# uber-research/vargp

Measured on AMD Instinct MI355X. Metric: ELBO steps/sec, higher is better.
Workload: dtype f32; 1 GPU; BASELINE config 2 (Split-MNIST t=0): S3 F10 C10 M100 D784 B512 ELBO step; S_per_gpu=3, Mt=100, S_total=3, F=10, C=10, M=100, D=784, B=512, N=12000, optimizer=yogi, parallelism=sample-parallel x1, steps_per_graph_launch=10, launch=hipGraph replay

## Files before the change

vargp_amd/csrc/elbo_t0.hip:

```cpp
#include <atomic>
#include <mutex>
#include <unordered_map>

#include "common.h"
STEP_SPAN_TABLE(t0)
#include "elbo_shared.h"
#include "t0_bwd_mid.h"
#include "t0_bwd_mid_multi.h"
#include "chol_gram.h"
#include "t0_prologue.h"
#include "t0_bwd_tail.h"

namespace vargp {

constexpr int kKuuSplit = 2;
#ifndef VARGP_KL_ROWS
#define VARGP_KL_ROWS 8
#endif
constexpr int kT0TileUnitsMax = 16384;
constexpr int kTailLdsDefault = 1;
constexpr int kKlRows = VARGP_KL_ROWS;


struct T0Ws {
  float* queue;
  float *theta, *eps_theta, *eps_f, *w, *g2, *kd, *na, *nb, *xs, *Lu, *KS, *LL, *TT, *RK, *QP, *W, *mu, *var;
  float *gmu, *gvar;
  float *r_uf, *c_uf, *gtheta;
  float *r_uu, *gW, *gkd, *gQP, *gLL, *gTT, *gRK, *gKS, *Wuu, *Puu, *Puf;
  float* kpart;
  void* chol;
  size_t chol_bytes;
  int NR, LD;
  int64_t Dp;
  size_t bytes;
};

static T0Ws carve_t0(void* ws, int S, int C, int M, int D, int B, int F) {
  T0Ws o{};
  o.NR = (int)round_up(4 + 2 * M, 4);
  o.LD = (int)round_up(o.NR + B, 4);
  o.Dp = round_up(D, 4);
  const int64_t SC = (int64_t)S * C, MM = (int64_t)M * M, D1 = D + 1;
  float* p = reinterpret_cast<float*>(ws);
  auto take = [&](int64_t n) { float* q = p; p += round_up(n, 64); return q; };
  o.theta = take(S * D1); o.eps_theta = take(S * D1); o.eps_f = take((int64_t)S * F * C * B);
  o.w = take(S * o.Dp); o.g2 = take(S); o.kd = take(SC); o.queue = take(8);
  o.na = take(SC * M); o.nb = take((int64_t)S * B);
  o.xs = take((int64_t)S * B * D);
  o.Lu = take(C * MM); o.KS = take((SC + C) * MM); o.LL = take((SC + C) * MM); o.TT = take((SC + C) * MM);
  o.RK = take(SC * M * o.LD); o.QP = take(SC * M * o.LD); o.W = take(SC * M * B);
  o.mu = take(SC * B); o.var = take(SC * B);
  o.gmu = take(SC * B); o.gvar = take(SC * B);
  o.r_uf = take(SC * M); o.c_uf = take((int64_t)S * B); o.gtheta = take(S * D1);
  o.r_uu = take(SC * M); o.gW = take(SC * M * B); o.gkd = take(SC);
  o.gQP = take(SC * M * o.LD); o.gLL = take((SC + C) * MM); o.gTT = take((SC + C) * MM);
  o.gRK = take(SC * M * o.LD); o.gKS = take((SC + C) * MM); o.Wuu = take(SC * MM);
  o.Puu = take(SC * M * D); o.Puf = take(SC * M * D);
  o.kpart = o.gRK;
  const size_t cb = vargp_chol_workspace_bytes((int)(SC + C), M, 0), cbb = vargp_chol_workspace_bytes((int)(SC + C), M, 1);
  o.chol_bytes = cb > cbb ? cb : cbb;
  o.chol = p;
  p += round_up((int64_t)(o.chol_bytes + 3) / 4, 64);
  o.bytes = (size_t)((char*)p - (char*)ws);
  return o;
}

__global__ __launch_bounds__(256) void t0_prologue_kernel(const ProArgs a) {
  __shared__ float red[4];
  t0_prologue_body(a, blockIdx.x, red);
}

__global__ __launch_bounds__(256) void t0_norm_kernel(const float* __restrict__ z, const float* __restrict__ x,
                                                      const float* __restrict__ w, float* __restrict__ na,
                                                      float* __restrict__ nb, int64_t zrows, int64_t xrows, int D,
                                                      int64_t Dp) {
  const int64_t row = (int64_t)blockIdx.x * 4 + (threadIdx.x >> 6);
  const int s = blockIdx.y, lane = threadIdx.x & 63;
  if (row >= zrows + xrows) return;
  const bool isz = row < zrows;
  const float* xr = isz ? z + row * D : x + (row - zrows) * D;
  const float* ws = w + s * Dp;
  const float acc = row_norm_wave(xr, ws, D, lane);
  if (lane == 0) {
    if (isz) na[(int64_t)s * zrows + row] = acc; else nb[(int64_t)s * xrows + (row - zrows)] = acc;
  }
}

__global__ __launch_bounds__(256) void t0_combine_norm_kernel(const float* __restrict__ part, int nsplit, int64_t sSplit,
                                                              const float* __restrict__ g2, float* __restrict__ Kuu, int C,
                                                              int M, int64_t total, int ncomb, const float* __restrict__ z,
                                                              const float* __restrict__ x, const float* __restrict__ w,
                                                              float* __restrict__ na, float* __restrict__ nb,
                                                              int64_t zrows, int64_t xrows, int D, int64_t Dp, int nrow4) {
  if ((int)blockIdx.x < ncomb) {
    const int64_t e = (int64_t)blockIdx.x * 256 + threadIdx.x;
    if (e >= total) return;
    const int j = e % M, i = (e / M) % M;
    const int64_t b = e / ((int64_t)M * M);
    const int64_t base = b * M * M;
    float gij = 0.f, gii = 0.f, gjj = 0.f;
    for (int k0 = 0; k0 < nsplit; k0 += 4) {
      float vij[4], vii[4], vjj[4];
#pragma unroll
      for (int q = 0; q < 4; ++q) {
        const float* pk = part + min(k0 + q, nsplit - 1) * sSplit + base;
        vij[q] = pk[(int64_t)i * M + j]; vii[q] = pk[(int64_t)i * M + i]; vjj[q] = pk[(int64_t)j * M + j];
      }
#pragma unroll
      for (int q = 0; q < 4; ++q) {
        if (k0 + q < nsplit) { gij += vij[q]; gii += vii[q]; gjj += vjj[q]; }
      }
    }
    const float gam = g2[b / C];
    Kuu[e] = i == j ? gam : gam * expf(-0.5f * (gii + gjj - 2.f * gij));
    return;
  }
  const int id = (int)blockIdx.x - ncomb;
  const int64_t row = (int64_t)(id % nrow4) * 4 + (threadIdx.x >> 6);
  const int s = id / nrow4, lane = threadIdx.x & 63;
  if (row >= zrows + xrows) return;
  const bool isz = row < zrows;
  const float* xr = isz ? z + row * D : x + (row - zrows) * D;
  const float* ws = w + s * Dp;
  const float acc = row_norm_wave(xr, ws, D, lane);
  if (lane == 0) {
    if (isz) na[(int64_t)s * zrows + row] = acc; else nb[(int64_t)s * xrows + (row - zrows)] = acc;
  }
}

__global__ void t0_pack_kernel(const float* __restrict__ m, const float* __restrict__ LS, const float* __restrict__ Lu,
                               float* __restrict__ RK, int C, int M, int NR, int LD, int64_t total) {
  const int64_t e = (int64_t)blockIdx.x * blockDim.x + threadIdx.x;
  if (e >= total) return;
  const int col = e % NR;
  const int64_t row = e / NR;
  const int i = row % M;
  const int64_t c = (row / M) % C;
  float v = 0.f;
  if (col == 0) v = m[c * M + i];
  else if (col >= 4 && col < 4 + M) v = LS[(c * M + i) * M + (col - 4)];
  else if (col >= 4 + M && col < 4 + 2 * M) v = Lu[(c * M + i) * M + (col - 4 - M)];
  RK[row * LD + col] = v;
}

__global__ __launch_bounds__(256) void t0_pdiag_kl_fwd_kernel(const float* __restrict__ QP, const float* __restrict__ W,
                                                              const float* __restrict__ kd, const float* __restrict__ Lz,
                                                              const float* __restrict__ Lu, float* __restrict__ mu,
                                                              float* __restrict__ var, float* __restrict__ kl_u, int S,
                                                              int C, int M, int B, int NR, int LD, int nbx, int npd,
                                                              int nkx, uint32_t* rng_counter) {
  __shared__ float red[3][4][64];
  if (rng_counter && blockIdx.x == 0 && threadIdx.x == 0) rng_counter[0] += 1u;
  if ((int)blockIdx.x < npd) {
    const int cx = threadIdx.x & 63, ry = threadIdx.x >> 6;
    const int col = ((int)blockIdx.x % nbx) * 64 + cx;
    const int64_t b = blockIdx.x / nbx;
    float m0 = 0.f, d1 = 0.f, d2 = 0.f;
    if (col < B) {
      const float* q = QP + b * M * LD;
      const float* p = q + NR + col;
      const float* w = W + b * M * B + col;
#pragma unroll 4
      for (int m = ry; m < M; m += 4) {
        const float pv = p[(int64_t)m * LD], wv = w[(int64_t)m * B];
        m0 = fmaf(pv, q[(int64_t)m * LD], m0);
        d1 = fmaf(pv, pv, d1);
        d2 = fmaf(wv, wv, d2);
      }
    }
    red[0][ry][cx] = m0; red[1][ry][cx] = d1; red[2][ry][cx] = d2;
    __syncthreads();
    if (ry == 0 && col < B) {
      m0 = red[0][0][cx] + red[0][1][cx] + red[0][2][cx] + red[0][3][cx];
      d1 = red[1][0][cx] + red[1][1][cx] + red[1][2][cx] + red[1][3][cx];
      d2 = red[2][0][cx] + red[2][1][cx] + red[2][2][cx] + red[2][3][cx];
      mu[b * B + col] = m0;
      var[b * B + col] = kd[b] - d1 + d2;
    }
    return;
  }
  const int id = (int)blockIdx.x - npd;
  const int64_t b = id / nkx;
  const int c = b % C;
  const int i0 = (id % nkx) * kKlRows, i1 = min(M, i0 + kKlRows);
  const float* q = QP + b * M * LD;
  float acc = 0.f;
  for (int e = threadIdx.x; e < (i1 - i0) * M; e += 256) {
    const int i = i0 + e / M, j = e % M;
    if (j <= i) { const float v = q[(int64_t)i * LD + 4 + M + j]; acc = fmaf(v, v, acc); }
  }
  for (int i = i0 + threadIdx.x; i < i1; i += 256) {
    const float a = q[(int64_t)i * LD];
    acc = fmaf(a, a, acc);
    acc += 2.f * (logf(Lz[(b * M + i) * M + i]) - logf(Lu[((int64_t)c * M + i) * M + i])) - 1.f;
  }
  const float t = block_sum<256>(acc, &red[0][0][0]);
  if (threadIdx.x == 0) atomicAdd(kl_u, 0.5f * t / (float)S);
}

constexpr int kFusedTS = 108;
constexpr int kFusedGS = 132;
constexpr int kFusedKS = 68;
constexpr int kFusedK = 104;
constexpr size_t kFusedLdsBytes = sizeof(float) * (128 * kFusedTS + kFusedK * kFusedGS + kFusedK * kFusedKS + 128 + 3 * 64);
typedef float f32x16_t __attribute__((ext_vector_type(16)));
#ifdef FF_STAMPS
__device__ unsigned long long g_ff_stamps[4][16];
extern "C" void vargp_debug_ff_stamps(unsigned long long* out) { (void)hipMemcpyFromSymbol(out, HIP_SYMBOL(g_ff_stamps), sizeof(g_ff_stamps)); }
#ifndef FF_STAMP_BLOCK
#define FF_STAMP_BLOCK 0u
#endif
#define FF_STAMP(i) do { if ((threadIdx.x & 63) == 0 && blockIdx.x == (FF_STAMP_BLOCK)) g_ff_stamps[threadIdx.x >> 6][i] = __builtin_amdgcn_s_memtime(); } while (0)
#else
#define FF_STAMP(i) do { } while (0)
#endif

__device__ __forceinline__ void ff_mfma4x2(f32x16_t& x, f32x16_t& y, const float4 a, const float4 c, const float4 b) {
  x = __builtin_amdgcn_mfma_f32_32x32x2f32(a.x, b.x, x, 0, 0, 0);
  y = __builtin_amdgcn_mfma_f32_32x32x2f32(c.x, b.x, y, 0, 0, 0);
  x = __builtin_amdgcn_mfma_f32_32x32x2f32(a.y, b.y, x, 0, 0, 0);
  y = __builtin_amdgcn_mfma_f32_32x32x2f32(c.y, b.y, y, 0, 0, 0);
  x = __builtin_amdgcn_mfma_f32_32x32x2f32(a.z, b.z, x, 0, 0, 0);
  y = __builtin_amdgcn_mfma_f32_32x32x2f32(c.z, b.z, y, 0, 0, 0);
  x = __builtin_amdgcn_mfma_f32_32x32x2f32(a.w, b.w, x, 0, 0, 0);
  y = __builtin_amdgcn_mfma_f32_32x32x2f32(c.w, b.w, y, 0, 0, 0);
}
__device__ __forceinline__ void ff_mfma4(f32x16_t& x, const float4 a, const float4 b) {
  x = __builtin_amdgcn_mfma_f32_32x32x2f32(a.x, b.x, x, 0, 0, 0);
  x = __builtin_amdgcn_mfma_f32_32x32x2f32(a.y, b.y, x, 0, 0, 0);
  x = __builtin_amdgcn_mfma_f32_32x32x2f32(a.z, b.z, x, 0, 0, 0);
  x = __builtin_amdgcn_mfma_f32_32x32x2f32(a.w, b.w, x, 0, 0, 0);
}
template <int R0, int R1>
__device__ __forceinline__ void ff_product_p(f32x16_t (&acc)[2], const float* __restrict__ sT, const float* __restrict__ sK, int cb,
                                             int li, int lh) {
  constexpr int GE = kFusedK / 8, G0 = bm_min(GE, 4 * R0 + 4), G1 = bm_min(GE, 4 * R1 + 4);
  const float* arow0 = sT + (32 * R0 + li) * kFusedTS + 4 * lh;
  const float* arow1 = sT + (32 * R1 + li) * kFusedTS + 4 * lh;
  const float* bcol = sK + (4 * lh) * kFusedKS + 32 * cb + li;
  float4 a0 = bm_frag_kc(arow0, 0), a1 = bm_frag_kc(arow1, 0), bb = bm_frag_km(bcol, 0, kFusedKS);
  bm_for<0, G1>([&](auto gi) {
    constexpr int g = decltype(gi)::value;
    const float4 c0 = a0, c1 = a1, cbv = bb;
    if constexpr (g + 1 < G1) {
      if constexpr (g + 1 < G0) a0 = bm_frag_kc(arow0, 8 * (g + 1));
      a1 = bm_frag_kc(arow1, 8 * (g + 1));
      bb = bm_frag_km(bcol, 8 * (g + 1), kFusedKS);
    }
    if constexpr (g < G0) ff_mfma4x2(acc[0], acc[1], c0, c1, cbv);
    else ff_mfma4(acc[1], c1, cbv);
  });
}
template <int R0, int R1>
__device__ __forceinline__ void ff_product_w(f32x16_t (&acc)[2], const float* __restrict__ sG, const float* __restrict__ sK, int cb,
                                             int li, int lh) {
  constexpr int GE = kFusedK / 8, S0 = 4 * R0, S1 = 4 * R1;
  const float* acol0 = sG + (4 * lh) * kFusedGS + 32 * R0 + li;
  const float* acol1 = sG + (4 * lh) * kFusedGS + 32 * R1 + li;
  const float* bcol = sK + (4 * lh) * kFusedKS + 32 * cb + li;
  float4 a0 = bm_frag_km(acol0, 8 * S0, kFusedGS), a1 = a0, bb = bm_frag_km(bcol, 8 * S0, kFusedKS);
  bm_for<S0, GE>([&](auto gi) {
    constexpr int g = decltype(gi)::value;
    const float4 c0 = a0, c1 = a1, cbv = bb;
    if constexpr (g + 1 < GE) {
      a0 = bm_frag_km(acol0, 8 * (g + 1), kFusedGS);
      if constexpr (g + 1 >= S1) a1 = bm_frag_km(acol1, 8 * (g + 1), kFusedGS);
      bb = bm_frag_km(bcol, 8 * (g + 1), kFusedKS);
    }
    if constexpr (g >= S1) ff_mfma4x2(acc[0], acc[1], c0, c1, cbv);
    else ff_mfma4(acc[0], c0, cbv);
  });
}

template <bool MULTI>
__device__ __forceinline__ void ff_barrier() {
  if constexpr (MULTI) bmm_lds_barrier(); else __syncthreads();
}
template <bool VEC4, bool MULTI = false>
__global__ __launch_bounds__(256) void t0_fwd_fused_kernel(const float* __restrict__ TT, float* __restrict__ QP,
                                                           const float* __restrict__ RK, float* __restrict__ W,
                                                           const float* __restrict__ kd, const float* __restrict__ Lz,
                                                           const float* __restrict__ Lu, float* __restrict__ mu,
                                                           float* __restrict__ var, float* __restrict__ kl_u, int S, int C,
                                                           int M, int B, int NR, int LD, int ntile, uint32_t* rng_counter,
                                                           int nparts) {
  extern __shared__ __attribute__((aligned(16))) float lds_f[];
  STEP_SPAN(t0, 3);
  float* sT = lds_f;
  float* sG = sT + 128 * kFusedTS;
  float* sK = sG + kFusedK * kFusedGS;
  float* sa = sK + kFusedK * kFusedKS;
  float* red = sa + 128;
  const int tid = threadIdx.x, lane = tid & 63, wave = tid >> 6, li = lane & 31, lh = lane >> 5;
  const int xcd = (int)blockIdx.x & 7, idx = (int)blockIdx.x >> 3;
  const int64_t b = (int64_t)(idx / nparts) * 8 + xcd;
  const int64_t MM = (int64_t)M * M, MLD = (int64_t)M * LD;
  if (rng_counter && blockIdx.x == 0 && tid == 0) rng_counter[0] += 1u;
  if (b >= (int64_t)S * C) return;
  const int part = idx % nparts;
  int tile_x = MULTI ? (part * ntile) / nparts : part;
  const int tile_end = MULTI ? ((part + 1) * ntile) / nparts : part + 1;
  int n0 = tile_x * 64;
  const float* Tb = TT + b * MM;
  const float* Qb = QP + b * MLD;
  const float* Kb = RK + b * MLD + NR;
  FF_STAMP(0);
  FF_STAMP(1);
  constexpr int NT_ = 128 * (kFusedK / 4) / 256;
  constexpr int NG_ = kFusedK * 32 / 256;
  constexpr int NK_ = (kFusedK * 16 + 255) / 256;
  float4 rt[NT_], rg[NG_], rk[NK_];
  const char* Tbb = reinterpret_cast<const char*>(Tb);
  const char* Qbb = reinterpret_cast<const char*>(Qb);
  const char* Kbb = reinterpret_cast<const char*>(Kb);
#pragma unroll
  for (int u = 0; u < NT_; ++u) {
    const int e = tid + 256 * u;
    const int i = e / (kFusedK / 4), k = (e - i * (kFusedK / 4)) * 4;
    const int ic = min(i, M - 1);
    rt[u] = *reinterpret_cast<const float4*>(Tbb + 4u * (__umul24((unsigned)ic, (unsigned)M) + (unsigned)min(k, min(M - 4, ic & ~3))));
  }
#pragma unroll
  for (int u = 0; u < NG_; ++u) {
    const int e = tid + 256 * u;
    const int k = e >> 5, i = (e & 31) * 4;
    const int kc = min(k, M - 1);
    rg[u] = *reinterpret_cast<const float4*>(Qbb + 4u * (__umul24((unsigned)kc, (unsigned)LD) + 4u + (unsigned)min(i, min(M - 4, kc & ~3))));
  }
  auto load_ktile = [&](const int n0_) {
    const char* Kt = Kbb + 4 * n0_;
#pragma unroll
    for (int u = 0; u < NK_; ++u) {
      const int e = min(tid + 256 * u, kFusedK * 16 - 1);
      const int k = e >> 4, n = (e & 15) * 4;
      const unsigned ro = 4u * __umul24((unsigned)min(k, M - 1), (unsigned)LD);
      if constexpr (VEC4) {
        rk[u] = *reinterpret_cast<const float4*>(Kt + ro + 4u * (unsigned)min(n, B - 4 - n0_));
      } else {
        const float* src = reinterpret_cast<const float*>(Kt + ro);
        rk[u].x = n0_ + n < B ? src[n] : 0.f;         rk[u].y = n0_ + n + 1 < B ? src[n + 1] : 0.f;
        rk[u].z = n0_ + n + 2 < B ? src[n + 2] : 0.f; rk[u].w = n0_ + n + 3 < B ? src[n + 3] : 0.f;
      }
    }
  };
  load_ktile(n0);
  const float av = tid < 128 ? *reinterpret_cast<const float*>(Qbb + 4u * __umul24((unsigned)min(tid, M - 1), (unsigned)LD)) : 0.f;
  const int c_kl = b % C;
  const int per = (M + nparts - 1) / nparts, i0 = part * per, i1 = min(M, i0 + per);
  const int nkl = max((i1 - i0) * M, 0);
  const unsigned mdiv = ((1u << 20) + (unsigned)M - 1u) / (unsigned)M;
  float kv[8];
#pragma unroll
  for (int u = 0; u < 8; ++u) {
    const int e = min(tid + 256 * u, max(nkl - 1, 0));
    const int ei = (int)(((unsigned)e * mdiv) >> 20);
    kv[u] = *reinterpret_cast<const float*>(Qbb + 4u * (__umul24((unsigned)min(i0 + ei, M - 1), (unsigned)LD) + 4u + (unsigned)M + (unsigned)(e - ei * M)));
  }
  const int idg = min(i0 + tid, M - 1);
  const float dga = *reinterpret_cast<const float*>(Qbb + 4u * __umul24((unsigned)idg, (unsigned)LD));
  const float dlz = Lz[(b * M + idg) * M + idg], dlu = Lu[((int64_t)c_kl * M + idg) * M + idg];
  FF_STAMP(10);
#pragma unroll
  for (int u = 0; u < NT_; ++u) {
    const int e = tid + 256 * u;
    const int i = e / (kFusedK / 4), k = (e - i * (kFusedK / 4)) * 4;
    const bool ok = i < M && k < M && k <= i;
    *reinterpret_cast<float4*>(&sT[i * kFusedTS + k]) = ok ? rt[u] : make_float4(0.f, 0.f, 0.f, 0.f);
  }
  FF_STAMP(11);
#pragma unroll
  for (int u = 0; u < NG_; ++u) {
    const int e = tid + 256 * u;
    const int k = e >> 5, i = (e & 31) * 4;
    *reinterpret_cast<float4*>(&sG[k * kFusedGS + i]) = (k < M && i < M && i <= k) ? rg[u] : make_float4(0.f, 0.f, 0.f, 0.f);
  }
  if (tid < 128) sa[tid] = tid < M ? av : 0.f;
  if (tid < 192) red[tid] = 0.f;
  float kl_acc = 0.f;
#pragma unroll
  for (int u = 0; u < 8; ++u) {
    const int e = tid + 256 * u;
    const int ei = (int)(((unsigned)e * mdiv) >> 20);
    const int i = i0 + ei, j = e - ei * M;
    kl_acc = fmaf((e < nkl && j <= i) ? kv[u] : 0.f, kv[u], kl_acc);
  }
  for (int e0 = 8 * 256; e0 < nkl; e0 += 8 * 256) {
#pragma unroll
    for (int u = 0; u < 8; ++u) {
      const int e = min(e0 + tid + 256 * u, nkl - 1);
      kv[u] = Qb[(int64_t)(i0 + e / M) * LD + 4 + M + e % M];
    }
#pragma unroll
    for (int u = 0; u < 8; ++u) {
      const int e = e0 + tid + 256 * u;
      const int i = i0 + e / M, j = e % M;
      kl_acc = fmaf((e < nkl && j <= i) ? kv[u] : 0.f, kv[u], kl_acc);
    }
  }
  {
    const bool dok = i0 + tid < i1;
    float t = fmaf(dga, dga, 2.f * (logf(dlz) - logf(dlu)) - 1.f);
    kl_acc += dok ? t : 0.f;
    for (int i = i0 + tid + 256; i < i1; i += 256) {
      const float a = Qb[(int64_t)i * LD];
      kl_acc = fmaf(a, a, kl_acc);
      kl_acc += 2.f * (logf(Lz[(b * M + i) * M + i]) - logf(Lu[((int64_t)c_kl * M + i) * M + i])) - 1.f;
    }
  }
  do {
#pragma unroll
  for (int u = 0; u < NK_; ++u) {
    const int e = tid + 256 * u;
    if (e < kFusedK * 16) {
      const int k = e >> 4, n = (e & 15) * 4;
      *reinterpret_cast<float4*>(&sK[k * kFusedKS + n]) = (k < M && (!VEC4 || n0 + n < B)) ? rk[u] : make_float4(0.f, 0.f, 0.f, 0.f);
    }
  }
  FF_STAMP(12);
  if constexpr (MULTI) { if (tile_x + 1 < tile_end) load_ktile(n0 + 64); }
  FF_STAMP(13);
  ff_barrier<MULTI>();
  FF_STAMP(2);
  if constexpr (MULTI) {
    const int l16 = lane & 15, q = lane >> 4, n = 16 * wave + l16, col = n0 + n;
    bm_f32x4 accP[kB16NB];
#pragma unroll
    for (int i = 0; i < kB16NB; ++i)
#pragma unroll
      for (int r = 0; r < 4; ++r) accP[i][r] = 0.f;
    b16_prod<true, kFusedTS>(sT, sK, wave, l16, q, accP);
    ff_barrier<true>();
    float s_mu = 0.f, s_p2 = 0.f, s_w2 = 0.f;
    char* Pout_b = reinterpret_cast<char*>(QP + b * MLD + NR);
#pragma unroll
    for (int i = 0; i < kB16NB; ++i) {
      float sav[4];
#pragma unroll
      for (int r = 0; r < 4; ++r) sav[r] = sa[16 * i + 4 * q + r];
#pragma unroll
      for (int r = 0; r < 4; ++r) {
        const int m = 16 * i + 4 * q + r;
        const float v = m < M ? accP[i][r] : 0.f;
        if (m < kFusedK) sK[m * kFusedKS + n] = v;
        if (m < M && col < B) *reinterpret_cast<float*>(Pout_b + 4u * (__umul24((unsigned)m, (unsigned)LD) + (unsigned)col)) = v;
        s_mu = fmaf(v, sav[r], s_mu);
        s_p2 = fmaf(v, v, s_p2);
      }
    }
    ff_barrier<true>();
    char* Wb_b = reinterpret_cast<char*>(W + b * (int64_t)M * B);
    bm_f32x4 accW[kB16NB];
#pragma unroll
    for (int i = 0; i < kB16NB; ++i)
#pragma unroll
      for (int r = 0; r < 4; ++r) accW[i][r] = 0.f;
    b16_prod<false, kFusedGS>(sG, sK, wave, l16, q, accW);
#pragma unroll
    for (int i = 0; i < kB16NB; ++i)
#pragma unroll
      for (int r = 0; r < 4; ++r) {
        const int m = 16 * i + 4 * q + r;
        if (m < M) {
          const float v = accW[i][r];
          if (col < B) *reinterpret_cast<float*>(Wb_b + 4u * (__umul24((unsigned)m, (unsigned)B) + (unsigned)col)) = v;
          s_w2 = fmaf(v, v, s_w2);
        }
      }
    s_mu += __shfl_xor(s_mu, 16, 64); s_p2 += __shfl_xor(s_p2, 16, 64); s_w2 += __shfl_xor(s_w2, 16, 64);
    s_mu += __shfl_xor(s_mu, 32, 64); s_p2 += __shfl_xor(s_p2, 32, 64); s_w2 += __shfl_xor(s_w2, 32, 64);
    if (q == 0) { red[n] = s_mu; red[64 + n] = s_p2; red[128 + n] = s_w2; }
    ff_barrier<true>();
    if (tid < 64 && n0 + tid < B) {
      mu[b * B + n0 + tid] = red[tid];
      var[b * B + n0 + tid] = kd[b] - red[64 + tid] + red[128 + tid];
    }
    tile_x += 1; n0 += 64;
  } else {
  const int cb = wave & 1;
  const int rbs[2] = {(wave >> 1) ? 1 : 0, (wave >> 1) ? 2 : 3};
  f32x16_t accP[2];
#pragma unroll
  for (int u = 0; u < 2; ++u)
#pragma unroll
    for (int r = 0; r < 16; ++r) accP[u][r] = 0.f;
  if ((wave >> 1) == 0) ff_product_p<0, 3>(accP, sT, sK, cb, li, lh);
  else ff_product_p<1, 2>(accP, sT, sK, cb, li, lh);
  FF_STAMP(3);
  ff_barrier<MULTI>();
  FF_STAMP(4);
  const int col = n0 + 32 * cb + li;
  float s_mu = 0.f, s_p2 = 0.f, s_w2 = 0.f;
  char* Pout_b = reinterpret_cast<char*>(QP + b * MLD + NR);
#pragma unroll
  for (int u = 0; u < 2; ++u) {
    float sav[16];
#pragma unroll
    for (int r = 0; r < 16; ++r) sav[r] = sa[32 * rbs[u] + (r & 3) + 8 * (r >> 2) + 4 * lh];
#pragma unroll
    for (int r = 0; r < 16; ++r) {
      const int m = 32 * rbs[u] + (r & 3) + 8 * (r >> 2) + 4 * lh;
      const float v = accP[u][r];
      if (m < kFusedK) sK[m * kFusedKS + 32 * cb + li] = v;
      if (m < M && col < B) *reinterpret_cast<float*>(Pout_b + 4u * (__umul24((unsigned)m, (unsigned)LD) + (unsigned)col)) = v;
      s_mu = fmaf(v, sav[r], s_mu);
      s_p2 = fmaf(v, v, s_p2);
    }
  }
  ff_barrier<MULTI>();
  FF_STAMP(5);
  char* Wb_b = reinterpret_cast<char*>(W + b * (int64_t)M * B);
  {
    const int rlo = min(rbs[0], rbs[1]), rhi = max(rbs[0], rbs[1]);
    f32x16_t accW[2];
#pragma unroll
    for (int u = 0; u < 2; ++u)
#pragma unroll
      for (int r = 0; r < 16; ++r) accW[u][r] = 0.f;
    if ((wave >> 1) == 0) ff_product_w<0, 3>(accW, sG, sK, cb, li, lh);
    else ff_product_w<1, 2>(accW, sG, sK, cb, li, lh);
    FF_STAMP(6);
#pragma unroll
    for (int u = 0; u < 2; ++u) {
      const int rb = u ? rhi : rlo;
#pragma unroll
      for (int r = 0; r < 16; ++r) {
        const int m = 32 * rb + (r & 3) + 8 * (r >> 2) + 4 * lh;
        if (m < M) {
          const float v = accW[u][r];
          if (col < B) *reinterpret_cast<float*>(Wb_b + 4u * (__umul24((unsigned)m, (unsigned)B) + (unsigned)col)) = v;
          s_w2 = fmaf(v, v, s_w2);
        }
      }
    }
  }
  FF_STAMP(7);
  s_mu += __shfl_xor(s_mu, 32, 64); s_p2 += __shfl_xor(s_p2, 32, 64); s_w2 += __shfl_xor(s_w2, 32, 64);
  if (lh == 0) {
    atomicAdd(&red[32 * cb + li], s_mu); atomicAdd(&red[64 + 32 * cb + li], s_p2); atomicAdd(&red[128 + 32 * cb + li], s_w2);
  }
  ff_barrier<MULTI>();
  if (tid < 64) {
    if (n0 + tid < B) {
      mu[b * B + n0 + tid] = red[tid];
      var[b * B + n0 + tid] = kd[b] - red[64 + tid] + red[128 + tid];
    }
  }
  FF_STAMP(8);
  }
  } while (MULTI && tile_x < tile_end);
  __syncthreads();
  const float tkl = block_sum<256>(kl_acc, red);
  if (tid == 0) atomicAdd(kl_u, 0.5f * tkl / (float)S);
  FF_STAMP(9);
}

__global__ __launch_bounds__(256) void t0_bwd_head_kernel(const float* __restrict__ QP, const float* __restrict__ W,
                                                          const float* __restrict__ gmu, const float* __restrict__ gvar,
                                                          const float* __restrict__ gscale, const float* __restrict__ Lz,
                                                          const float* __restrict__ seeds, float* __restrict__ gQP,
                                                          float* __restrict__ gW, float* __restrict__ gkd,
                                                          float* __restrict__ gLz, float* __restrict__ gThead,
                                                          float* __restrict__ gTtail, float* __restrict__ zero_begin, int64_t zero_count, int S, int C,
                                                          int M, int B, int NR, int LD, int npd, int nkx, int nkl, int fused,
                                                          float* __restrict__ g_u_mean, float* __restrict__ gLu_acc) {
  __shared__ float red[4];
  const float g = seeds[1] / (float)S;
  if ((int)blockIdx.x < npd) {
    const int m = (int)blockIdx.x % M;
    const int64_t b = blockIdx.x / M;
    const int64_t offp = (b * M + m) * LD + NR, offw = (b * M + m) * B;
    const float am = QP[(b * M + m) * LD];
    const float gs = gscale ? gscale[0] : 1.f;
    float acc = 0.f, accv = 0.f;
    for (int c0 = 0; c0 < B; c0 += 1024) {
      float gm[4], gv[4], pv[4], wv[4];
#pragma unroll
      for (int q = 0; q < 4; ++q) {
        const int col = min(c0 + 256 * q + (int)threadIdx.x, B - 1);
        gm[q] = gmu[b * B + col]; gv[q] = gvar[b * B + col];
        pv[q] = QP[offp + col]; wv[q] = W[offw + col];
      }
#pragma unroll
      for (int q = 0; q < 4; ++q) {
        const int col = c0 + 256 * q + (int)threadIdx.x;
        if (col < B) {
          const float m_ = gs * gm[q], v_ = gs * gv[q];
          gQP[offp + col] = am * m_ - 2.f * pv[q] * v_;
          gW[offw + col] = 2.f * wv[q] * v_;
          acc = fmaf(pv[q], m_, acc);
          accv += v_;
        }
      }
    }
    const float t = block_sum<256>(acc, red);
    if (threadIdx.x == 0) gQP[(b * M + m) * LD] = t + g * am;
    if (m == 0) {
      const float tv = block_sum<256>(accv, red);
      if (threadIdx.x == 0) gkd[b] = tv;
    }
    return;
  }
  const int id = (int)blockIdx.x - npd;
  if (id >= nkl) {
    const int nz = gridDim.x - npd - nkl;
    for (int64_t i = (int64_t)(id - nkl) * 256 + threadIdx.x; i < zero_count; i += (int64_t)nz * 256) zero_begin[i] = 0.f;
    return;
  }
  const int64_t b = id / nkx;
  const int s = b / C, c = b % C;
  const int i0 = (id % nkx) * kKlRows, i1 = min(M, i0 + kKlRows);
  const float* q = QP + b * M * LD;
  float* gq = gQP + b * M * LD;
  const int nel = (i1 - i0) * M;
  for (int e00 = 0; e00 < nel; e00 += 1024) {
    float qv[4], lv[4];
#pragma unroll
    for (int u = 0; u < 4; ++u) {
      const int e0 = min(e00 + 256 * u + (int)threadIdx.x, nel - 1);
      const int i = i0 + e0 / M, j = e0 % M;
      qv[u] = q[(int64_t)i * LD + 4 + M + j];
      lv[u] = Lz[b * M * M + i * M + j];
    }
#pragma unroll
    for (int u = 0; u < 4; ++u) {
      const int e0 = e00 + 256 * u + (int)threadIdx.x;
      if (e0 < nel) {
        const int i = i0 + e0 / M, j = e0 % M;
        const int e = i * M + j;
        gq[(int64_t)i * LD + 4 + M + j] = (j <= i) ? g * qv[u] : 0.f;
        gq[(int64_t)i * LD + 4 + j] = 0.f;
        gThead[b * M * M + e] = 0.f;
        gLz[b * M * M + e] = (i == j) ? g / lv[u] : 0.f;
        if (s == 0) {
          gTtail[(int64_t)c * M * M + e] = 0.f;
          if (gLu_acc) gLu_acc[(int64_t)c * M * M + e] = 0.f;
        }
      }
    }
  }
  for (int i = i0 + threadIdx.x; i < i1; i += 256) {
    if (fused) gq[(int64_t)i * LD] = g * q[(int64_t)i * LD];
    if (g_u_mean && s == 0) g_u_mean[(int64_t)c * M + i] = 0.f;
    gq[(int64_t)i * LD + 1] = 0.f; gq[(int64_t)i * LD + 2] = 0.f; gq[(int64_t)i * LD + 3] = 0.f;
    for (int col = 4 + 2 * M; col < NR; ++col) gq[(int64_t)i * LD + col] = 0.f;
  }
  if (fused && i0 == 0 && threadIdx.x == 0) gkd[b] = 0.f;
}

__global__ void t0_unpack_kernel(const float* __restrict__ gRK, float* __restrict__ g_u_mean, float* __restrict__ gLS,
                                 int S, int C, int M, int LD, int64_t total) {
  const int64_t e = (int64_t)blockIdx.x * blockDim.x + threadIdx.x;
  if (e >= total) return;
  const int jj = e % (M + 1);
  const int64_t ci = e / (M + 1);
  const int col = jj == 0 ? 0 : 3 + jj;
  float acc = 0.f;
  for (int s0 = 0; s0 < S; s0 += 8) {
    float t[8];
#pragma unroll
    for (int u = 0; u < 8; ++u) t[u] = gRK[((int64_t)min(s0 + u, S - 1) * C * M + ci) * LD + col];
#pragma unroll
    for (int u = 0; u < 8; ++u) acc += (s0 + u < S) ? t[u] : 0.f;
  }
  if (jj == 0) g_u_mean[ci] = acc; else gLS[ci * M + (jj - 1)] = acc;
}

static int ensure_dynamic_lds(const void* fn, size_t bytes, std::atomic<unsigned> (&mask)[2], const char* who) {
  int dev = 0;
  VARGP_REQUIRE(hipGetDevice(&dev) == hipSuccess && dev >= 0 && dev < 64, "%s: hipGetDevice failed", who);
  if (!((mask[dev >> 5].load(std::memory_order_acquire) >> (dev & 31)) & 1u)) {
    VARGP_REQUIRE(hipFuncSetAttribute(fn, hipFuncAttributeMaxDynamicSharedMemorySize, (int)bytes) == hipSuccess,
                  "%s: cannot reserve %zu bytes of LDS", who, bytes);
    mask[dev >> 5].fetch_or(1u << (dev & 31), std::memory_order_release);
  }
  return VARGP_OK;
}

static bool t0_native(const vargp_elbo_t0_desc* d) { return d->eps_f == nullptr && !d->ext_lik; }
static int check_desc(const vargp_elbo_t0_desc* d, const char* who) {
  VARGP_REQUIRE(d, "%s: null descriptor", who);
  VARGP_REQUIRE(d->S > 0 && d->C > 0 && d->M > 0 && d->D > 0 && d->B > 0 && d->F > 0, "%s: bad dims", who);
  VARGP_REQUIRE(d->log_mean && d->z && d->u_mean && d->u_tril_vec && d->x && (d->y || d->ext_lik) && d->scalars && d->info && d->ws,
                "%s: null pointer", who);
  const bool native = t0_native(d);
  VARGP_REQUIRE(!native || (d->rng_counter && d->eps_theta == nullptr && d->rng_sample_offset >= 0),
                "%s: native noise needs rng_counter, eps_theta == eps_f == NULL and a sample offset >= 0", who);
  VARGP_REQUIRE(d->map_est ? d->S == 1
                           : (d->log_logvar && d->prior_log_mean && d->prior_log_logvar && (native || d->eps_theta)),
                "%s: hyper-parameter arguments inconsistent with map_est", who);
  VARGP_REQUIRE(d->ws_bytes >= vargp_elbo_t0_workspace_bytes(d->S, d->C, d->M, d->D, d->B, d->F),
                "%s: workspace too small", who);
  return VARGP_OK;
}

struct T0Tune {
  static long long env(const char* name, long long dflt) { const char* e = getenv(name); return e ? atoll(e) : dflt; }
  int64_t units = env("VARGP_T0_UNITS", kT0TileUnitsMax);
  int unmerge = env("VARGP_T0_UNMERGE", -1), side = env("VARGP_T0_SIDE", 1);
  int multi = env("VARGP_T0_MULTI", 0), parts = env("VARGP_T0_PARTS", 0);
  int fused = env("VARGP_T0_FUSED", 1), fused_bwd = env("VARGP_T0_FUSED_BWD", 1), mat_bwd = env("VARGP_T0_MAT_BWD", 1);
  int front = env("VARGP_T0_FRONT", 1), gram_in_chain = env("VARGP_T0_GRAM_IN_CHAIN", -1), su = env("VARGP_T0_SU", 1);
  int tail = env("VARGP_T0_TAIL", 1), tail_lds = env("VARGP_T0_TAIL_LDS", kTailLdsDefault);
  int kuf_tile = env("VARGP_T0_KUF_TILE", 0), puf_tile = env("VARGP_T0_PUF_TILE", 0), puu_tile = env("VARGP_T0_PUU_TILE", 0);
  int kuu_split = env("VARGP_KUU_SPLIT", kKuuSplit), chol_f32 = env("VARGP_CHOL_F32", kCholF32Default);
};
static const T0Tune& t0_tune() { static const T0Tune tune; return tune; }

constexpr float kFwdMidSetup = 0.5f;
constexpr float kBwdMidSetup = 0.35f;
static int t0_tile_parts(int64_t SC, int ntile, int cus, float setup, int forced) {
  if (forced > 0) return forced < ntile ? forced : ntile;
  if (SC * ntile <= cus) return ntile;
  int best = ntile;
  float best_t = 1e30f;
  for (int np = 1; np <= ntile; ++np) {
    const float t = (float)cdiv(SC * np, (int64_t)cus) * (setup + (float)cdiv(ntile, np));
    if (t < best_t - 1e-6f) { best_t = t; best = np; }
  }
  return best;
}

struct T0Plan {
  bool native, generic_lik, unscaled_lik_grad, defer_softmax, fwd_softmax16;
  bool direct_gram, merge_chol, split_kuu, front, gram_in_chain, su_in_chain, fused_mid, fwd_multi, w_vec4;
  bool unmerge, side;
  bool fused_bwd, mat_bwd, bwd_multi, fused_tail, tail_lds;
  int kuf_tile, puf_tile, puu_tile;
  int ksp, ntile, fwd_parts, bwd_parts;
};
static T0Plan t0_plan(const vargp_elbo_t0_desc* d, const T0Ws& o, int cus) {
  const T0Tune& tune = t0_tune();
  const int S = d->S, C = d->C, M = d->M, D = d->D, B = d->B, F = d->F, LD = o.LD;
  const int64_t SC = (int64_t)S * C;
  const bool zx_aligned = ((reinterpret_cast<uintptr_t>(d->z) | reinterpret_cast<uintptr_t>(d->x)) & 15) == 0;
  T0Plan p{};
  p.native = t0_native(d);
  p.unscaled_lik_grad = C <= 16 && !d->ext_lik;
  p.generic_lik = C > 16 && !d->ext_lik;
  p.ntile = cdiv(B, 64);
  p.kuf_tile = tune.kuf_tile; p.puf_tile = tune.puf_tile; p.puu_tile = tune.puu_tile;

  p.direct_gram = D <= kRbfDirectD;
  p.merge_chol = D > kRbfDirectD && M > 50 && M <= 100 && (D % 4) == 0 && (LD % 4) == 0 && zx_aligned;
  p.ksp = tune.kuu_split;
  p.split_kuu = p.merge_chol && D >= 256 && (int64_t)p.ksp * M <= LD && p.ksp > 1;
  p.front = p.split_kuu && tune.front && p.ksp <= kCholPartMax && D <= kProKuuMaxD;

  p.unmerge = SC + C >= (tune.unmerge >= 0 ? tune.unmerge : cus / 3 + 1);
  p.side = p.unmerge && tune.side != 0;

  p.gram_in_chain = p.front && (tune.gram_in_chain >= 0 ? S >= tune.gram_in_chain : p.unmerge) && M > 64 && (M % 4) == 0 &&
                    D <= kCgMaxD && D >= 32;
  p.su_in_chain = VARGP_CHOL_BLK16 && tune.su && tune.chol_f32 && p.merge_chol && M > 64 && (M % 4) == 0 && M <= 100;

  const bool units_ok = SC * p.ntile <= tune.units;
  p.fused_mid = tune.fused && M <= kFusedK && (M % 4) == 0 && (LD % 4) == 0 && units_ok;
  p.fwd_parts = t0_tile_parts(SC, p.ntile, cus, kFwdMidSetup, tune.parts);
  p.fwd_multi = p.fwd_parts < p.ntile || tune.multi == 1;
  p.w_vec4 = B % 4 == 0;
  p.fused_bwd = tune.fused_bwd && M <= kBmKP && M >= 4 && (M % 4) == 0 && (LD % 4) == 0 && (B % 4) == 0 && units_ok;
  p.mat_bwd = p.fused_bwd && tune.mat_bwd && (D % 4) == 0 && S <= kTailSMax && zx_aligned;
  p.bwd_parts = t0_tile_parts(SC, p.ntile, cus, kBwdMidSetup, tune.parts);
  p.bwd_multi = p.fused_bwd && (p.bwd_parts < p.ntile || tune.multi == 1);
  p.defer_softmax = d->defer_softmax && p.unscaled_lik_grad && p.fused_bwd && !p.bwd_multi && F <= 4 * kBmSmF && C <= kBmSmC &&
                    reinterpret_cast<uintptr_t>(p.native ? o.eps_f : d->eps_f) % 16 == 0;
  p.fwd_softmax16 = p.unscaled_lik_grad && !p.defer_softmax;
  p.fused_tail = p.mat_bwd && tune.tail && S <= kTailSMax;
  p.tail_lds = p.fused_tail && ((S > 4 && tune.tail_lds) || tune.tail_lds == 2);
  return p;
}

enum { kT0NoClear = 0, kT0Cleared = 1, kT0Consumed = 2, kT0SoftmaxDeferred = 16  };
static std::mutex g_t0_state_mu;
static std::unordered_map<const void*, int> g_t0_state;
static void t0_state_set(const void* ws, int v) {
  std::lock_guard<std::mutex> lock(g_t0_state_mu);
  if (g_t0_state.size() > 4096) {
    for (auto it = g_t0_state.begin(); it != g_t0_state.end();)
      it = ((it->second & 15) == kT0Cleared && it->first != ws) ? std::next(it) : g_t0_state.erase(it);
  }
  g_t0_state[ws] = v;
}
static int t0_state_get(const void* ws) {
  std::lock_guard<std::mutex> lock(g_t0_state_mu);
  auto it = g_t0_state.find(ws);
  return it == g_t0_state.end() ? -1 : it->second;
}

struct T0 {
  const vargp_elbo_t0_desc* d;
  T0Ws o;
  T0Plan plan;
  vargp_stream_t stream;
  hipStream_t st;
  int S, C, M, D, B, F, SC, NR, LD;
  int64_t MM, MLD, zrows;
  const float *eps_f, *eps_theta;

  T0(const vargp_elbo_t0_desc* d_, vargp_stream_t stream_)
      : d(d_), o(carve_t0(d_->ws, d_->S, d_->C, d_->M, d_->D, d_->B, d_->F)), plan(t0_plan(d_, o, vargp_cu_count())),
        stream(stream_), st(as_stream(stream_)), S(d_->S), C(d_->C), M(d_->M), D(d_->D), B(d_->B), F(d_->F), SC(d_->S * d_->C),
        NR(o.NR), LD(o.LD), MM((int64_t)d_->M * d_->M), MLD((int64_t)d_->M * o.LD), zrows((int64_t)d_->C * d_->M),
        eps_f(plan.native ? o.eps_f : d_->eps_f), eps_theta(plan.native ? o.eps_theta : d_->eps_theta) {}

  GemmParams kuu_gemm() const {
    GemmParams p = flat_gemm(d->z, D, 0, d->z, D, 0, o.KS, M, C * MM, M, M, D);
    p.nb1 = C; p.sA[1] = (int64_t)M * D; p.sB[1] = (int64_t)M * D; p.sC[1] = MM;
    p.kscale = o.w; p.ks_ld = o.Dp; p.g2 = o.g2;
    p.na = o.na; p.sNa[0] = zrows; p.sNa[1] = M;
    p.nbv = o.na; p.sNb[0] = zrows; p.sNb[1] = M;
    p.same_xy = 1;
    return p;
  }
  GemmParams kuf_gemm(bool prescaled) const {
    GemmParams p = flat_gemm(d->z, D, 0, d->x, D, 0, o.RK + NR, LD, (int64_t)C * MLD, C * M, B, D);
    p.kscale = o.w; p.ks_ld = o.Dp; p.g2 = o.g2;
    p.na = o.na; p.sNa[0] = zrows;
    p.nbv = o.nb; p.sNb[0] = B;
    if (prescaled) { p.B = o.xs; p.sB[0] = (int64_t)B * D; p.kscale = nullptr; }
    return p;
  }
  ElboGemm qp_gemm(int ncols) const {
    ElboGemm g{flat_gemm(o.TT, M, MM, o.RK, LD, MLD, o.QP, LD, MLD, M, ncols, M), 0, 0, SC, ncols == NR ? "t0_qps_gemm" : "t0_qp_gemm"};
    g.p.triA = 1;
    return g;
  }
  ElboGemm gt_gemm(bool small) const {
    ElboGemm g{flat_gemm(o.gQP, LD, MLD, o.RK, LD, MLD, o.gTT, M, MM, M, M, small ? NR : NR + B), 0, 1, SC, "t0_gt_gemm"};
    g.p.triC = 1;
    if (small) return g.onto_c();
    g.p.splitk = ksplit(NR + B);
    return g;
  }
  ElboGemm grk_gemm(int ncols) const {
    ElboGemm g{flat_gemm(o.TT, M, MM, o.gQP, LD, MLD, o.gRK, LD, MLD, M, ncols, M), 1, 0, SC, "t0_grk_gemm"};
    g.p.triA = 2;
    return g;
  }
  GemmParams puu_gemm() const {
    GemmParams p = flat_gemm(o.Wuu, M, C * MM, d->z, D, 0, o.Puu, D, zrows * D, M, D, M);
    p.nb1 = C; p.sA[1] = MM; p.sB[1] = (int64_t)M * D; p.sC[1] = (int64_t)M * D;
    return p;
  }
  GemmParams puf_gemm() const { return flat_gemm(o.gRK + NR, LD, C * MLD, d->x, D, 0, o.Puf, D, zrows * D, C * M, D, B); }
  int fwd() const;
  int bwd(const float* seeds, float* g_log_mean, float* g_log_logvar, float* g_z, float* g_u_mean, float* g_u_tril_vec) const;
};

int T0::fwd() const {
  int rc;
  t0_state_set(d->ws, (plan.mat_bwd ? kT0Cleared : kT0NoClear) | (plan.defer_softmax ? kT0SoftmaxDeferred : 0));
  ZeroJobs bwd_zero{};
  if (plan.mat_bwd) {
    bwd_zero.j[0] = ZeroJob{o.gQP, (int64_t)SC * M, 4 + M, LD};
    bwd_zero.j[1] = ZeroJob{o.gTT, 1, (SC + C) * MM, 0};
    bwd_zero.j[2] = ZeroJob{o.queue, 1, 8, 0};
    bwd_zero.j[3] = ZeroJob{o.gkd, 1, SC, 0};
    bwd_zero.j[4] = ZeroJob{o.r_uf, 1, o.r_uu - o.r_uf, 0};
    if (plan.unmerge)
      bwd_zero.j[5] = ZeroJob{o.gLL + SC * MM, 1, C * MM, 0};
  }
  ProArgs a{};
  if (plan.merge_chol) { a.RK = o.RK; a.u_mean = d->u_mean; a.NR = NR; a.LD = LD; }
  a.mean = d->log_mean; a.logvar = d->log_logvar; a.pmean = d->prior_log_mean; a.plogvar = d->prior_log_logvar;
  a.eps_theta = d->eps_theta; a.vec = d->u_tril_vec;
  a.theta = o.theta; a.w = o.w; a.g2 = o.g2; a.kd = o.kd; a.Lu = o.Lu; a.Su = o.KS + SC * MM; a.scalars = d->scalars;
  a.bump = d->bump;
  a.su_in_chain = plan.su_in_chain ? 1 : 0;
  a.zero_begin = o.gmu; a.zero_count = o.r_uf - o.gmu; a.info = d->info; a.Dp = o.Dp;
  a.S = S; a.C = C; a.M = M; a.D = D; a.ninfo = SC + C; a.map_est = d->map_est;
  a.nzero_blocks = (int)std::min<int64_t>(64, cdiv(a.zero_count, 1024));
  if (plan.native) {
    const int64_t per_sample_f = (int64_t)F * C * B;
    a.native = 1; a.seed = d->rng_seed; a.rng_counter = d->rng_counter;
    a.g0_theta = (int64_t)d->rng_sample_offset * (D + 1); a.g0_f = (int64_t)d->rng_sample_offset * per_sample_f;
    a.n_f = S * per_sample_f;
    a.eps_theta_out = o.eps_theta; a.eps_f_out = o.eps_f;
    a.nrng_blocks = (int)std::min<int64_t>(512, cdiv(a.n_f + 7, 1024));
  }
  if (plan.mat_bwd && !plan.merge_chol) {
    a.zero = bwd_zero;
    const int64_t zt = (int64_t)SC * M * (4 + M) + (SC + 2 * C) * MM + (o.r_uu - o.r_uf);
    a.nzero_blocks = (int)std::min<int64_t>(128, cdiv(a.zero_count + zt, 2048));
  }
  const int npro = 1 + S + a.nzero_blocks + a.nrng_blocks + cdiv((int64_t)C * MM, 256);
  if (!plan.front) {
    ProfScope prof("t0_prologue", st);
    hipLaunchKernelGGL(t0_prologue_kernel, dim3(npro), dim3(256), 0, st, a);
  }
  if (plan.direct_gram) {
    rc = rbf_direct_launch(d->z, nullptr, o.w, o.g2, o.KS, M, S, C, M, M, D, o.Dp, 0, st);
    if (rc) return rc;
    rc = rbf_direct_launch(d->z, d->x, o.w, o.g2, o.RK + NR, LD, S, C, M, B, D, o.Dp, 1, st);
    if (rc) return rc;
  } else {
    if (!plan.split_kuu)
      hipLaunchKernelGGL(t0_norm_kernel, dim3(cdiv(zrows + B, 4), S), dim3(256), 0, st, d->z, d->x, o.w, o.na, o.nb, zrows,
                         (int64_t)B, D, o.Dp);
    if (plan.merge_chol) {
      VARGP_REQUIRE(chol_rbf_gemm_applicable(M, kuf_gemm(false)), "elbo_t0_fwd: merged launch expected but not applicable");
      if (plan.split_kuu) {
        GemmParams ps = kuu_gemm();
        ps.splitk = plan.ksp; ps.sSplit = SC * MM; ps.C = o.kpart;
        if (plan.front) {
          NormArgs nr{d->z, d->x, o.na, o.nb, zrows, (int64_t)B, 16, (int)cdiv(zrows + B, 16), o.xs};
          rc = launch_pro_kuu(a, npro, nr, ps, plan.gram_in_chain ? 0 : SC, st);
          if (rc) return rc;
        } else {
          rc = launch_gemm(ps, 0, 1, SC, true, st, "rbf_kuu_gemm");
          if (rc) return rc;
          const int64_t total = SC * MM;
          const int ncomb = cdiv(total, 256), nrow4 = cdiv(zrows + B, 4);
          hipLaunchKernelGGL(t0_combine_norm_kernel, dim3(ncomb + nrow4 * S), dim3(256), 0, st, o.kpart, plan.ksp, SC * MM, o.g2,
                             o.KS, C, M, total, ncomb, d->z, d->x, o.w, o.na, o.nb, zrows, (int64_t)B, D, o.Dp, nrow4);
        }
      } else {
        rc = launch_gemm(kuu_gemm(), 0, 1, SC, true, st, "rbf_kuu_gemm");
        if (rc) return rc;
      }
      CholExtra lx{o.RK + 4, SC, LD, MLD, (int64_t)C * MLD, S, 1, 1};
      if (plan.front) {
        lx.part = o.kpart; lx.nsplit = plan.ksp; lx.sSplit = SC * MM; lx.g2 = o.g2; lx.part_C = C; lx.Kout = o.KS;
        if (plan.gram_in_chain) { lx.part = nullptr; lx.gram_z = d->z; lx.gram_w = o.w; lx.gram_D = D; lx.gram_Dp = o.Dp; }
      }
      if (plan.su_in_chain) lx.su_Lu = o.Lu;
      GemmParams kuf = kuf_gemm(plan.front);
      SideFork fork(st, plan.side);
      rc = launch_chol_rbf_gemm(o.KS, d->jitter, o.LL, o.TT, d->info, SC + C, M, kuf, plan.unmerge ? 0 : S, fork.side(), &lx,
                                plan.mat_bwd ? &bwd_zero : nullptr);
      if (rc) return rc;
      if (plan.unmerge) {
        kuf.tile = plan.kuf_tile;
        rc = launch_gemm(kuf, 0, 1, S, true, st, "rbf_kuf_gemm");
        if (rc) return rc;
      }
      rc = fork.join();
      if (rc) return rc;
    } else {
      rc = launch_gemm_pair(kuu_gemm(), SC, kuf_gemm(false), S, 0, 1, true, st, "rbf_kuu_gemm", "rbf_kuf_gemm");
      if (rc) return rc;
    }
  }
  if (!plan.merge_chol) {
    rc = chol_inv_fwd_impl(o.KS, d->jitter, o.LL, o.TT, nullptr, d->info, SC + C, M, o.chol, o.chol_bytes, false, st);
    if (rc) return rc;
    const int64_t total = (int64_t)SC * M * NR;
    hipLaunchKernelGGL(t0_pack_kernel, dim3(cdiv(total, 256)), dim3(256), 0, st, d->u_mean, o.LL + SC * MM, o.Lu, o.RK, C,
                       M, NR, LD, total);
  }
  if (d->info_host && d->info_event) {
    VARGP_REQUIRE(hipMemcpyAsync(d->info_host, d->info, sizeof(int32_t) * (size_t)(SC + C), hipMemcpyDeviceToHost, st) == hipSuccess &&
                      hipEventRecord(reinterpret_cast<hipEvent_t>(d->info_event), st) == hipSuccess,
                  "elbo_t0_fwd: copy / event record of the early Cholesky status failed");
  }
  uint32_t* rngc = plan.native ? d->rng_counter : nullptr;
  if (plan.fused_mid) {
    rc = qp_gemm(NR).run(st);
    if (rc) return rc;
    static std::atomic<unsigned> attr_set_mask[4][2] = {};
    const dim3 grid(8 * cdiv(SC, 8) * plan.fwd_parts);
#define VARGP_FF(V4, MT, SLOT)                                                                                                  \
  do {                                                                                                                          \
    rc = ensure_dynamic_lds(reinterpret_cast<const void*>(t0_fwd_fused_kernel<V4, MT>), kFusedLdsBytes, attr_set_mask[SLOT],    \
                            "elbo_t0_fwd");                                                                                     \
    if (rc) return rc;                                                                                                          \
    hipLaunchKernelGGL((t0_fwd_fused_kernel<V4, MT>), grid, dim3(256), kFusedLdsBytes, st, o.TT, o.QP, o.RK, o.W, o.kd, o.LL,   \
                       o.Lu, o.mu, o.var, d->scalars + 1, S, C, M, B, NR, LD, plan.ntile, rngc, plan.fwd_parts);                  \
  } while (0)
    if (plan.w_vec4) { if (plan.fwd_multi) VARGP_FF(true, true, 0); else VARGP_FF(true, false, 1); }
    else { if (plan.fwd_multi) VARGP_FF(false, true, 2); else VARGP_FF(false, false, 3); }
#undef VARGP_FF
  } else {
    rc = qp_gemm(NR + B).run(st);
    if (rc) return rc;
    ElboGemm w{flat_gemm(o.QP + 4, LD, MLD, o.QP + NR, LD, MLD, o.W, B, (int64_t)M * B, M, B, M), 1, 0, SC, "t0_w_gemm"};
    w.p.triA = 2;
    rc = w.run(st);
    if (rc) return rc;
    const int ntile = plan.ntile, npd = ntile * SC, nkx = cdiv(M, kKlRows);
    hipLaunchKernelGGL(t0_pdiag_kl_fwd_kernel, dim3(npd + nkx * SC), dim3(256), 0, st, o.QP, o.W, o.kd, o.LL, o.Lu, o.mu,
                       o.var, d->scalars + 1, S, C, M, B, NR, LD, ntile, npd, nkx, rngc);
  }
  if (plan.fwd_softmax16) {
    const int64_t total = (int64_t)S * F * B;
    hipLaunchKernelGGL(t0_softmax_kernel<16>, dim3(cdiv(total, 256)), dim3(256), 0, st, o.mu, o.var, eps_f, d->y,
                       d->scalars + 2, o.gmu, o.gvar, S, F, C, B);
  } else if (plan.generic_lik) {
    rc = vargp_softmax_nll_fwd(o.mu, o.var, eps_f, d->y, d->scalars + 2, S, F, C, B, stream);
    if (rc) return rc;
  }
  return check_launch("elbo_t0_fwd");
}

int T0::bwd(const float* seeds, float* g_log_mean, float* g_log_logvar, float* g_z, float* g_u_mean, float* g_u_tril_vec) const {
  int rc;
  const int64_t MB = (int64_t)M * B;
  const float* lik_seed = plan.unscaled_lik_grad ? seeds + 2 : nullptr;
  if (plan.generic_lik) {
    rc = vargp_softmax_nll_bwd(o.mu, o.var, eps_f, d->y, seeds + 2, o.gmu, o.gvar, S, F, C, B, stream);
    if (rc) return rc;
  }
  const int state_all = t0_state_get(d->ws);
  const bool softmax_deferred = state_all >= 0 && (state_all & kT0SoftmaxDeferred) != 0;
  VARGP_REQUIRE(!softmax_deferred || plan.fused_bwd, "elbo_t0_bwd: the forward deferred the likelihood to a backward path this call does not take");
  if (plan.mat_bwd) {
    const int state = state_all < 0 ? state_all : (state_all & ~kT0SoftmaxDeferred);
    VARGP_REQUIRE(state == kT0Cleared,
                  "elbo_t0_bwd: %s -- this path allows ONE vargp_elbo_t0_bwd per vargp_elbo_t0_fwd (the forward clears the "
                  "accumulators the backward adds into); run the forward again",
                  state == kT0Consumed ? "second backward on one forward"
                                       : "no forward on this workspace with the same z / x alignment");
    t0_state_set(d->ws, kT0Consumed);
  } else if (softmax_deferred) {
    t0_state_set(d->ws, kT0NoClear);
  }
  if (!plan.mat_bwd) {
    const int npd = plan.fused_bwd ? 0 : M * SC, nkx = cdiv(M, kKlRows), nkl = nkx * SC;
    const int64_t zc = o.r_uu - o.r_uf;
    const int nz = (int)std::min<int64_t>(64, cdiv(zc, 1024));
    hipLaunchKernelGGL(t0_bwd_head_kernel, dim3(npd + nkl + nz), dim3(256), 0, st, o.QP, o.W, o.gmu, o.gvar, lik_seed, o.LL,
                       seeds, o.gQP, o.gW, o.gkd, o.gLL, o.gTT, o.gTT + SC * MM, o.r_uf, zc, S, C, M, B, NR, LD, npd, nkx, nkl,
                       plan.fused_bwd ? 1 : 0, (float*)nullptr, (float*)nullptr);
  }
  if (plan.fused_bwd) {
    static std::atomic<unsigned> attr_set_mask[2] = {}, attr_set_mask_m[2] = {};
    float* gum = plan.mat_bwd ? g_u_mean : nullptr;
    if (plan.bwd_multi) {
      VARGP_REQUIRE(!softmax_deferred, "elbo_t0_bwd: the multi-tile backward does not evaluate a deferred likelihood");
      rc = ensure_dynamic_lds(reinterpret_cast<const void*>(t0_bwd_mid_multi_kernel), kBwdMidMultiLdsBytes, attr_set_mask_m, "elbo_t0_bwd");
      if (rc) return rc;
      ProfScope prof("t0_bwd_mid", st);
      hipLaunchKernelGGL(t0_bwd_mid_multi_kernel, dim3(8 * cdiv(SC, 8) * plan.bwd_parts), dim3(256), kBwdMidMultiLdsBytes, st, o.TT, o.QP,
                         o.W, o.RK, o.gmu, o.gvar, lik_seed, o.gQP, o.gTT, o.gRK, o.gkd, o.r_uf, o.c_uf, o.gtheta, S, C, M,
                         B, D, NR, LD, plan.ntile, plan.bwd_parts, gum, C * M);
    } else {
      const BmSoftmax smx = softmax_deferred ? BmSoftmax{o.mu, o.var, eps_f, d->y, d->scalars + 2, F} : BmSoftmax{};
      rc = ensure_dynamic_lds(reinterpret_cast<const void*>(t0_bwd_mid_kernel), kBwdMidLdsBytes, attr_set_mask, "elbo_t0_bwd");
      if (rc) return rc;
      ProfScope prof("t0_bwd_mid", st);
      hipLaunchKernelGGL(t0_bwd_mid_kernel, dim3(8 * cdiv(SC, 8) * plan.ntile), dim3(256), kBwdMidLdsBytes, st, o.TT, o.QP, o.W, o.RK, o.gmu, o.gvar,
                         lik_seed, o.gQP, o.gTT, o.gRK, o.gkd, o.r_uf, o.c_uf, o.gtheta, S, C, M, B, D,
                         NR, LD, plan.ntile, gum, C * M, smx);
    }
    if (!plan.mat_bwd) {
      rc = run_gemm_pair(gt_gemm(true), grk_gemm(NR), "t0_gt_grk_small", st);
      if (rc) return rc;
      rc = chol_inv_bwd_first(o.TT, o.gTT, SC + C, M, o.chol, o.chol_bytes, nullptr, 0, 0, 0, st);
      if (rc) return rc;
    }
  } else {
    ElboGemm gg{flat_gemm(o.QP + NR, LD, MLD, o.gW, B, MB, o.gQP + 4, LD, MLD, M, M, B), 0, 1, SC, "t0_gg_gemm"};
    gg.p.splitk = ksplit(B);
    ElboGemm gp{flat_gemm(o.QP + 4, LD, MLD, o.gW, B, MB, o.gQP + NR, LD, MLD, M, B, M), 0, 0, SC, "t0_gp_gemm"};
    gp.p.triA = 1;
    rc = run_gemm_pair(gg, gp.onto_c(), "t0_gg_gp_gemm", st);
    if (rc) return rc;
    rc = gt_gemm(false).run(st);
    if (rc) return rc;
    const ElboGemm grk = grk_gemm(NR + B);
    rc = chol_inv_bwd_first(o.TT, o.gTT, SC + C, M, o.chol, o.chol_bytes, &grk.p, grk.tA, grk.tB, grk.nbatch, st);
    if (rc) return rc;
  }
  if (plan.mat_bwd) {
    BwdMatArgs ma{};
    ma.QP = o.QP; ma.TT = o.TT; ma.LL = o.LL; ma.gQP = o.gQP; ma.RK = o.RK; ma.KS = o.KS; ma.seeds = seeds; ma.gTT = o.gTT;
    ma.gKS = o.gKS; ma.Wuu = o.Wuu; ma.r_uu = o.r_uu; ma.gtheta = o.gtheta;
    ma.g_u_mean = g_u_mean; ma.gLu_part = o.gLL;
    ma.S = S; ma.C = C; ma.M = M; ma.D = D; ma.NR = NR; ma.LD = LD;
    GemmParams puf = puf_gemm();
    if (plan.unmerge) {
      SideFork fork(st, plan.side);
      ma.gL_acc = o.gLL + SC * MM;
      rc = launch_bwdmat_gemm(ma, 0, SC, puf, 0, fork.side(), "t0_bwdmat_kuu", nullptr);
      if (rc) return rc;
      rc = launch_bwdmat_gemm(ma, SC, C, puf, 0, fork.side(), "t0_bwdmat_su", nullptr);
      if (rc) return rc;
      puf.tile = plan.puf_tile;
      rc = launch_gemm(puf, 0, 0, S, false, st, "rbf_kuf_bwd_product");
      if (rc) return rc;
      rc = fork.join();
    } else {
      rc = launch_bwdmat_gemm(ma, 0, SC + C, puf, S, st, "rbf_kuf_bwd_gemm", reinterpret_cast<int*>(o.queue));
    }
    if (rc) return rc;
    if (!plan.fused_tail) {
      GemmParams puu = puu_gemm();
      puu.tile = plan.puu_tile;
      rc = launch_gemm(puu, 0, 0, SC, false, st, "rbf_kuu_bwd_gemm");
      if (rc) return rc;
    }
  } else {
    const int64_t total = (int64_t)C * M * (M + 1);
    hipLaunchKernelGGL(t0_unpack_kernel, dim3(cdiv(total, 256)), dim3(256), 0, st, o.gRK, g_u_mean, o.gLL + SC * MM, S, C,
                       M, LD, total);
    rc = chol_inv_bwd_impl(o.LL, o.TT, o.gLL, o.gTT, o.gKS, SC + C, M, o.chol, o.chol_bytes, true, st, true);
    if (rc) return rc;
    const int gx = cdiv(B, 256), gy = cdiv(zrows, kWRows), nuf = plan.fused_bwd ? 0 : gx * gy * S;
    const int nuu = SC * cdiv(M, kUuRows);
    const int ngv = cdiv((int64_t)C * MM, 256);
    hipLaunchKernelGGL(t0_w_kernel, dim3(nuf + nuu + ngv), dim3(256), 0, st, o.RK, o.gRK, o.KS, o.gKS, o.Wuu, o.r_uu, o.r_uf,
                       o.c_uf, o.gtheta, S, C, M, B, D, NR, LD, gx, gy, nuf, nuu, d->u_tril_vec, o.Lu, seeds, g_u_tril_vec, 1);
    rc = launch_gemm_pair(puu_gemm(), SC, puf_gemm(), S, 0, 0, false, st, "rbf_kuu_bwd_gemm", "rbf_kuf_bwd_gemm");
    if (rc) return rc;
  }
  const int nzy = cdiv(zrows, kFinRows), nxy = cdiv(B, kFinRows), gx = cdiv(D, 64);
  GvecArgs gv{};
  int ngy = 0;
  if (plan.mat_bwd) {
    gv.vec = d->u_tril_vec; gv.Lu = o.Lu; gv.gSu = o.gKS + SC * MM; gv.gLu_part = o.gLL; gv.seeds = seeds;
    gv.gvec = g_u_tril_vec; gv.S = S; gv.C = C; gv.M = M; gv.y0 = nzy + nxy;
    ngy = cdiv(cdiv((int64_t)C * MM, 256), gx);
  }
  if (plan.fused_tail) {
    ProfScope prof("t0_puu_final", st);
    TailArgs ta{};
    ta.z = d->z; ta.x = d->x; ta.Wuu = o.Wuu; ta.Puf = o.Puf; ta.r_uu = o.r_uu; ta.r_uf = o.r_uf; ta.c_uf = o.c_uf; ta.w = o.w;
    ta.gz = g_z; ta.gtheta = o.gtheta; ta.S = S; ta.C = C; ta.M = M; ta.D = D; ta.B = B; ta.Dp = o.Dp;
    const int rem = M % 32;
    ta.nrb = (rem > 0 && rem <= 8) ? M / 32 : cdiv(M, 32);
    const int ngr = cdiv(M, 32);
    ta.ncb = cdiv(D, 32); ta.nz = cdiv(C * ta.nrb * ta.ncb + C * (ngr * (ngr + 1) / 2), 4);
    ta.nx = gx * cdiv(B, kTailXRows); ta.gx = gx;
    ta.nrem = (rem > 0 && rem <= 8) ? C * gx * cdiv(rem, 4) : 0;
    const dim3 grid(ta.nz + ta.nrem + ta.nx);
    if (plan.tail_lds) {
      static std::atomic<unsigned> attr_set_mask_t[2] = {};
      rc = ensure_dynamic_lds(reinterpret_cast<const void*>(t0_puu_final_lds_kernel), kTailLdsBytes, attr_set_mask_t, "elbo_t0_bwd");
      if (rc) return rc;
      const int nzg = C * ta.nrb * cdiv(ta.ncb, 4), ngvw = cdiv(C * (ngr * (ngr + 1) / 2), 4);
      hipLaunchKernelGGL(t0_puu_final_lds_kernel, dim3(nzg + ngvw + ta.nrem + ta.nx), dim3(512), kTailLdsBytes, st, ta, gv, nzg, ngvw);
    } else
    switch (S) {
      case 1: hipLaunchKernelGGL(t0_puu_final_kernel<1>, grid, dim3(256), 0, st, ta, gv); break;
      case 2: hipLaunchKernelGGL(t0_puu_final_kernel<2>, grid, dim3(256), 0, st, ta, gv); break;
      case 3: hipLaunchKernelGGL(t0_puu_final_kernel<3>, grid, dim3(256), 0, st, ta, gv); break;
      case 4: hipLaunchKernelGGL(t0_puu_final_kernel<4>, grid, dim3(256), 0, st, ta, gv); break;
      default: hipLaunchKernelGGL(t0_puu_final_kernel<0>, grid, dim3(256), 0, st, ta, gv); break;
    }
  } else {
    hipLaunchKernelGGL(t0_final_kernel, dim3(gx, nzy + nxy + ngy), dim3(256), 0, st, d->z, d->x, o.r_uu, o.r_uf, o.c_uf,
                       o.Puu, o.Puf, o.w, g_z, o.gtheta, zrows, (int64_t)B, D, o.Dp, S, nzy, gv);
  }
  if (!d->defer_hyper) {
    vargp_hyper_grad_desc h;
    hyper_grad_desc_fill(d, o, eps_theta, seeds, &h);
    hyper_bwd_launch(h, g_log_mean, g_log_logvar, st);
  }
  return check_launch("elbo_t0_bwd");
}

}

using namespace vargp;

extern "C" size_t vargp_elbo_t0_workspace_bytes(int S, int C, int M, int D, int B, int F) {
  return carve_t0(nullptr, S, C, M, D, B, F).bytes + 256;
}

extern "C" int vargp_elbo_t0_lik_buffers(const vargp_elbo_t0_desc* d, float** mu, float** var, float** gmu, float** gvar) {
  VARGP_REQUIRE(d && d->ws, "elbo_t0_lik_buffers: null pointer");
  const T0Ws o = carve_t0(d->ws, d->S, d->C, d->M, d->D, d->B, d->F);
  if (mu) *mu = o.mu;
  if (var) *var = o.var;
  if (gmu) *gmu = o.gmu;
  if (gvar) *gvar = o.gvar;
  return VARGP_OK;
}

extern "C" int vargp_elbo_t0_fwd(const vargp_elbo_t0_desc* d, vargp_stream_t stream) {
  const int rc = check_desc(d, "elbo_t0_fwd");
  return rc ? rc : T0(d, stream).fwd();
}

extern "C" int vargp_elbo_t0_bwd(const vargp_elbo_t0_desc* d, const float* seeds, float* g_log_mean, float* g_log_logvar,
                                 float* g_z, float* g_u_mean, float* g_u_tril_vec, vargp_stream_t stream) {
  const int rc = check_desc(d, "elbo_t0_bwd");
  if (rc) return rc;
  VARGP_REQUIRE(seeds && g_z && g_u_mean && g_u_tril_vec && (d->defer_hyper || (g_log_mean && g_log_logvar)),
                "elbo_t0_bwd: null pointer");
  return T0(d, stream).bwd(seeds, g_log_mean, g_log_logvar, g_z, g_u_mean, g_u_tril_vec);
}

extern "C" int vargp_elbo_t0_hyper_desc(const vargp_elbo_t0_desc* d, const float* seeds, vargp_hyper_grad_desc* out) {
  int rc = check_desc(d, "elbo_t0_hyper_desc");
  if (rc) return rc;
  VARGP_REQUIRE(seeds && out, "elbo_t0_hyper_desc: null pointer");
  const T0Ws o = carve_t0(d->ws, d->S, d->C, d->M, d->D, d->B, d->F);
  hyper_grad_desc_fill(d, o, t0_native(d) ? o.eps_theta : d->eps_theta, seeds, out);
  return VARGP_OK;
}
```

vargp_amd/csrc/t0_bwd_common.h:

```cpp
#pragma once
#include "common.h"
#include <type_traits>

namespace vargp {


constexpr int kBmKP = 104;
constexpr int kBmSA = 108;
constexpr int kBmST = 68;
constexpr size_t kBwdMidLdsBytes =
    sizeof(float) * (kBmKP * kBmSA + 2 * kBmKP * kBmST + 128  + 64 + 64  + 64  + 8 +
                     3 * 4 * 64 );
constexpr int kBmSmC = 16, kBmSmF = 4;
struct BmSoftmax {
  const float *mu, *var, *eps;
  const int64_t* y;
  float* nll;
  int F;
};
typedef float bm_f32x16 __attribute__((ext_vector_type(16)));

__device__ __forceinline__ float4 bm_frag_kc(const float* __restrict__ rowp, int k) {
  return *reinterpret_cast<const float4*>(rowp + k);
}
__device__ __forceinline__ float4 bm_frag_km(const float* __restrict__ colp, int k, int stride) {
  const float* p = colp + k * stride;
  return make_float4(p[0], p[stride], p[2 * stride], p[3 * stride]);
}
__device__ __forceinline__ void bm_mfma4(bm_f32x16& acc, const float4 a, const float4 b) {
  acc = __builtin_amdgcn_mfma_f32_32x32x2f32(a.x, b.x, acc, 0, 0, 0);
  acc = __builtin_amdgcn_mfma_f32_32x32x2f32(a.y, b.y, acc, 0, 0, 0);
  acc = __builtin_amdgcn_mfma_f32_32x32x2f32(a.z, b.z, acc, 0, 0, 0);
  acc = __builtin_amdgcn_mfma_f32_32x32x2f32(a.w, b.w, acc, 0, 0, 0);
}

__device__ __forceinline__ void bmm_lds_barrier() { asm volatile("s_waitcnt lgkmcnt(0)\n\ts_barrier" ::: "memory"); }

template <int I0, int I1, class F>
__device__ __forceinline__ void bm_for(F&& f) {
  if constexpr (I0 < I1) {
    f(std::integral_constant<int, I0>{});
    bm_for<I0 + 1, I1>(f);
  }
}
__host__ __device__ constexpr int bm_min(int a, int b) { return a < b ? a : b; }

constexpr int kBmNQ = kBmKP / 4;
constexpr int kBmNA = (kBmKP * kBmNQ + 255) / 256;

template <bool TRI = false>
__device__ __forceinline__ void bm_load_mat(const float* __restrict__ base, int ld, int M, int tid, float4 (&dst)[kBmNA]) {
  const char* bp = reinterpret_cast<const char*>(base);
#pragma unroll
  for (int u = 0; u < kBmNA; ++u) {
    const int e = min(tid + 256 * u, kBmKP * kBmNQ - 1);
    const int i = e / kBmNQ, j = (e - i * kBmNQ) * 4;
    const int ic = min(i, M - 1);
    const int jc = TRI ? min(j, min(M - 4, ic & ~3)) : min(j, M - 4);
    const unsigned off = 4u * (__umul24((unsigned)ic, (unsigned)ld) + (unsigned)jc);
    dst[u] = *reinterpret_cast<const float4*>(bp + off);
  }
}

}
```

vargp_amd/csrc/t0_bwd_mid.h:

```cpp
#pragma once
#include "t0_bwd_common.h"

namespace vargp {

template <int WV> struct BmWave {
  static constexpr int NB = WV < 2 ? 3 : 2;
  static constexpr int R0 = WV < 2 ? 0 : 1, R1 = WV < 2 ? 3 : 2, CBH = WV & 1;
  __host__ __device__ static constexpr int rb(int u) { return WV == 0 ? (u == 0 ? 0 : 1) : (WV == 1 ? 2 : 3); }
  __host__ __device__ static constexpr int cb(int u) { return WV == 0 ? (u == 2 ? 1 : 0) : (WV == 1 ? u : (WV == 2 ? u : 2 + u)); }
};

__host__ __device__ constexpr int kBmAtomSplit(int nb) { return 8 * nb; }

template <int WV>
__device__ __forceinline__ void bm_tri_mfma(const float* __restrict__ sX, const float* __restrict__ sY, int li, int lh,
                                            bm_f32x16 (&acc)[3]) {
  using W = BmWave<WV>;
  const float* xr[3];
  const float* yr[3];
#pragma unroll
  for (int u = 0; u < 3; ++u) {
#pragma unroll
    for (int r = 0; r < 16; ++r) acc[u][r] = 0.f;
    xr[u] = sX + min(32 * W::rb(u < W::NB ? u : 0) + li, kBmKP - 1) * kBmST + 4 * lh;
    yr[u] = sY + min(32 * W::cb(u < W::NB ? u : 0) + li, kBmKP - 1) * kBmST + 4 * lh;
  }
#pragma unroll
  for (int k = 0; k < 64; k += 8) {
#pragma unroll
    for (int u = 0; u < W::NB; ++u) bm_mfma4(acc[u], bm_frag_kc(xr[u], k), bm_frag_kc(yr[u], k));
  }
}
template <int WV, int A>
__device__ __forceinline__ void bm_tri_atomic(const bm_f32x16 (&acc)[3], float* __restrict__ dst, int ldd, int M, int li, int lh) {
  using W = BmWave<WV>;
  constexpr int u = A / 16, r = A % 16, rb = W::rb(u), cb = W::cb(u);
  constexpr int rl = (r & 3) + 8 * (r >> 2);
  if (32 * rb + rl < M) {
    const int row = 32 * rb + rl + 4 * lh, col = 32 * cb + li;
    const bool ok = row < M && (rb != cb || col <= row);
#ifndef BM_EXP_NOATOM
#ifdef BM_EXP_PLAIN_STORES
    if (ok) dst[(int64_t)row * ldd + col] = acc[u][r];
#else
    if (ok) atomicAdd(&dst[(int64_t)row * ldd + col], acc[u][r]);
#endif
#else
    if (ok && acc[u][r] == 12345.f) dst[(int64_t)row * ldd + col] = 0.f;
#endif
  }
}

template <int WV>
__device__ __forceinline__ void bm_phase2(const float* __restrict__ sA, const float* __restrict__ sP, const float* __restrict__ sW,
                                          const float* __restrict__ sa, const float* __restrict__ sgm,
                                          const float* __restrict__ sgv, float* __restrict__ dst, int ldd, int M, int li, int lh,
                                          bm_f32x16 (&accP)[2], bm_f32x16 (&acc)[3]) {
  using W = BmWave<WV>;
  bm_tri_mfma<WV>(sP, sW, li, lh, acc);
  constexpr int R[2] = {W::R0, W::R1};
  const int n = 32 * W::CBH + li;
  {
    const float gmn = sgm[n], gvn = sgv[n];
#pragma unroll
    for (int u = 0; u < 2; ++u)
#pragma unroll
      for (int r = 0; r < 16; ++r) {
        const int m = 32 * R[u] + (r & 3) + 8 * (r >> 2) + 4 * lh;
        const int mc = min(m, kBmKP - 1);
        accP[u][r] = m < kBmKP ? fmaf(sa[mc], gmn, -2.f * sP[mc * kBmST + n] * gvn) : 0.f;
      }
  }
  constexpr int G0 = bm_min(kBmKP, 32 * W::R0 + 32) / 8, G1 = bm_min(kBmKP, 32 * W::R1 + 32) / 8;
  constexpr int NAT = kBmAtomSplit(W::NB), PER = (NAT + G1 - 1) / G1;
  const float* arow0 = sA + min(32 * W::R0 + li, kBmKP - 1) * kBmSA + 4 * lh;
  const float* arow1 = sA + min(32 * W::R1 + li, kBmKP - 1) * kBmSA + 4 * lh;
  const float* bcol = sW + (4 * lh) * kBmST + n;
  float4 nb = bm_frag_km(bcol, 0, kBmST), na0 = bm_frag_kc(arow0, 0), na1 = bm_frag_kc(arow1, 0);
  bm_for<0, G1>([&](auto gi) {
    constexpr int g = decltype(gi)::value;
    const float4 bb = nb, a0 = na0, a1 = na1;
    if constexpr (g + 1 < G1) {
      nb = bm_frag_km(bcol, 8 * (g + 1), kBmST);
      na1 = bm_frag_kc(arow1, 8 * (g + 1));
      if constexpr (g + 1 < G0) na0 = bm_frag_kc(arow0, 8 * (g + 1));
    }
    bm_mfma4(accP[1], a1, bb);
    if constexpr (g < G0) bm_mfma4(accP[0], a0, bb);
    bm_for<g * PER, bm_min((g + 1) * PER, NAT)>([&](auto ai) { bm_tri_atomic<WV, decltype(ai)::value>(acc, dst, ldd, M, li, lh); });
    __builtin_amdgcn_sched_barrier(0);
  });
}

template <int WV>
__device__ __forceinline__ void bm_phase4(const float* __restrict__ sA, const float* __restrict__ sP, const float* __restrict__ sW,
                                          float* __restrict__ dst, int ldd, int M, int li, int lh, bm_f32x16 (&accK)[2],
                                          const bm_f32x16 (&prev)[3], float* __restrict__ dprev, int ldprev, bm_f32x16 (&acc)[3]) {
  using W = BmWave<WV>;
  {
    const float* xr[3];
    const float* yr[3];
#pragma unroll
    for (int u = 0; u < 3; ++u) {
#pragma unroll
      for (int r = 0; r < 16; ++r) acc[u][r] = 0.f;
      xr[u] = sP + min(32 * W::rb(u < W::NB ? u : 0) + li, kBmKP - 1) * kBmST + 4 * lh;
      yr[u] = sW + min(32 * W::cb(u < W::NB ? u : 0) + li, kBmKP - 1) * kBmST + 4 * lh;
    }
    constexpr int A0 = kBmAtomSplit(W::NB), A1 = 16 * W::NB, PERP = (A1 - A0 + 7) / 8;
    bm_for<0, 8>([&](auto gi) {
      constexpr int g = decltype(gi)::value;
#pragma unroll
      for (int u = 0; u < W::NB; ++u) bm_mfma4(acc[u], bm_frag_kc(xr[u], 8 * g), bm_frag_kc(yr[u], 8 * g));
      bm_for<A0 + g * PERP, bm_min(A0 + (g + 1) * PERP, A1)>(
          [&](auto ai) { bm_tri_atomic<WV, decltype(ai)::value>(prev, dprev, ldprev, M, li, lh); });
    });
  }
#pragma unroll
  for (int u = 0; u < 2; ++u)
#pragma unroll
    for (int r = 0; r < 16; ++r) accK[u][r] = 0.f;
  constexpr int GS0 = 4 * W::R0, GS1 = 4 * W::R1, GE = kBmKP / 8;
  constexpr int NIT = GE - GS0, NAT = kBmAtomSplit(W::NB), PER = (NAT + NIT - 1) / NIT;
  const int n = 32 * W::CBH + li;
  const float* acol0 = sA + (4 * lh) * kBmSA + min(32 * W::R0 + li, kBmKP - 1);
  const float* acol1 = sA + (4 * lh) * kBmSA + min(32 * W::R1 + li, kBmKP - 1);
  const float* bcol = sP + (4 * lh) * kBmST + n;
  float4 nb = bm_frag_km(bcol, 8 * GS0, kBmST), na0 = bm_frag_km(acol0, 8 * GS0, kBmSA), na1 = na0;
  if constexpr (GS1 == GS0) na1 = bm_frag_km(acol1, 8 * GS0, kBmSA);
  bm_for<GS0, GE>([&](auto gi) {
    constexpr int g = decltype(gi)::value;
    const float4 bb = nb, a0 = na0, a1 = na1;
    if constexpr (g + 1 < GE) {
      nb = bm_frag_km(bcol, 8 * (g + 1), kBmST);
      na0 = bm_frag_km(acol0, 8 * (g + 1), kBmSA);
      if constexpr (g + 1 >= GS1) na1 = bm_frag_km(acol1, 8 * (g + 1), kBmSA);
    }
    bm_mfma4(accK[0], a0, bb);
    if constexpr (g >= GS1) bm_mfma4(accK[1], a1, bb);
    constexpr int it = g - GS0;
    bm_for<it * PER, bm_min((it + 1) * PER, NAT)>([&](auto ai) { bm_tri_atomic<WV, decltype(ai)::value>(acc, dst, ldd, M, li, lh); });
    __builtin_amdgcn_sched_barrier(0);
  });
}

template <int WV>
__device__ __forceinline__ void bm_tail_atomics(const bm_f32x16 (&acc)[3], float* __restrict__ dst, int ldd, int M, int li, int lh) {
  using W = BmWave<WV>;
  bm_for<kBmAtomSplit(W::NB), 16 * W::NB>([&](auto ai) { bm_tri_atomic<WV, decltype(ai)::value>(acc, dst, ldd, M, li, lh); });
}

#ifdef BM_STAMPS
__device__ unsigned long long g_bm_stamps[16];
extern "C" void vargp_debug_bm_stamps(unsigned long long* out) { (void)hipMemcpyFromSymbol(out, HIP_SYMBOL(g_bm_stamps), 128); }
#ifndef BM_STAMP_BLOCK
#define BM_STAMP_BLOCK 0u
#endif
#define BM_STAMP(i) do { if (threadIdx.x == 0 && blockIdx.x == (BM_STAMP_BLOCK)) g_bm_stamps[i] = __builtin_amdgcn_s_memtime(); } while (0)
#else
#define BM_STAMP(i) do { } while (0)
#endif
#ifdef BM_CUT
#define BM_CUT_AT(i) do { if (BM_CUT == (i)) return; } while (0)
#else
#define BM_CUT_AT(i) do { } while (0)
#endif

constexpr int kBmNT = (kBmKP * 16 + 255) / 256;

__device__ __forceinline__ void bm_load_tile(const float* __restrict__ base, int ld, int M, int n0, int B, int tid,
                                             float4 (&dst)[kBmNT]) {
  const char* bp = reinterpret_cast<const char*>(base);
#pragma unroll
  for (int u = 0; u < kBmNT; ++u) {
    const int e = min(tid + 256 * u, kBmKP * 16 - 1);
    const int m = e >> 4, n = (e & 15) * 4;
    const unsigned off = 4u * (__umul24((unsigned)min(m, M - 1), (unsigned)ld) + (unsigned)min(n0 + n, B - 4));
    dst[u] = *reinterpret_cast<const float4*>(bp + off);
  }
}
__device__ __forceinline__ void bm_store_tile(float* __restrict__ dst, const float4 (&src)[kBmNT], int M, int n0, int B, int tid) {
#pragma unroll
  for (int u = 0; u < kBmNT; ++u) {
    const int e = tid + 256 * u;
    const int m = e >> 4, n = (e & 15) * 4;
    const float4 v = (m < M && n0 + n < B) ? src[u] : make_float4(0.f, 0.f, 0.f, 0.f);
    if (e < kBmKP * 16) *reinterpret_cast<float4*>(&dst[m * kBmST + n]) = v;
  }
}

template <bool TRI = false>
__device__ __forceinline__ void bm_store_mat(float* __restrict__ dst, const float4 (&src)[kBmNA], int M, int tid) {
#pragma unroll
  for (int u = 0; u < kBmNA; ++u) {
    const int e = tid + 256 * u;
    const int i = e / kBmNQ, j = (e - i * kBmNQ) * 4;
    const float4 v = (i < M && j < M && (!TRI || j <= i)) ? src[u] : make_float4(0.f, 0.f, 0.f, 0.f);
    if (e < kBmKP * kBmNQ) *reinterpret_cast<float4*>(&dst[i * kBmSA + j]) = v;
  }
}

__global__ __launch_bounds__(256) void t0_bwd_mid_kernel(const float* __restrict__ TT, const float* __restrict__ QP,
                                                         const float* __restrict__ Wf, const float* __restrict__ RK,
                                                         const float* __restrict__ gmu, const float* __restrict__ gvar,
                                                         const float* __restrict__ gscale, float* __restrict__ gQP,
                                                         float* __restrict__ gTT, float* __restrict__ gRK,
                                                         float* __restrict__ gkd, float* __restrict__ r_uf,
                                                         float* __restrict__ c_uf, float* __restrict__ gtheta, int S, int C,
                                                         int M, int B, int D, int NR, int LD, int ntile,
                                                         float* __restrict__ zero_out, int zero_n, const BmSoftmax sm) {
  extern __shared__ __attribute__((aligned(16))) float bm_lds[];
  STEP_SPAN(t0, 4);
  if (blockIdx.x == 0 && zero_out)
    for (int i = threadIdx.x; i < zero_n; i += 256) zero_out[i] = 0.f;
  float* sA = bm_lds;
  float* sP = sA + kBmKP * kBmSA;
  float* sW = sP + kBmKP * kBmST;
  float* sa = sW + kBmKP * kBmST;
  float* sgm = sa + 128;
  float* sgv = sgm + 64;
  float* scs = sgv + 64;
  const int tid = threadIdx.x, lane = tid & 63, wave = tid >> 6, li = lane & 31, lh = lane >> 5;
  const int xcd = (int)blockIdx.x & 7, idx = (int)blockIdx.x >> 3;
  const int64_t b = (int64_t)(idx / ntile) * 8 + xcd;
  if (b >= (int64_t)S * C) return;
  const int n0 = (idx % ntile) * 64;
  const int64_t MM = (int64_t)M * M, MLD = (int64_t)M * LD;
  const float* Qb = QP + b * MLD;
  const float* Tb = TT + b * MM;
  const float* Wb = Wf + b * (int64_t)M * B;
  const float* Kb = RK + b * MLD + NR;
  const float gs = gscale ? gscale[0] : 1.f;
  constexpr int NA_ = kBmNA, NT_ = kBmNT;
  BM_STAMP(0);
  const int q4 = tid & 15, fs = tid >> 4;
  const int nq = min(n0 + 4 * q4, B - 4);
  float4 sev[kBmSmC], mu4 = make_float4(0.f, 0.f, 0.f, 0.f), var4 = mu4;
  int64_t yq[4] = {0, 0, 0, 0};
  if (sm.eps) {
    const int s = (int)(b / C);
    const int64_t rc = ((int64_t)s * C + min(fs, C - 1)) * B + nq;
    mu4 = *reinterpret_cast<const float4*>(sm.mu + rc);
    var4 = *reinterpret_cast<const float4*>(sm.var + rc);
    const float* ep = sm.eps + ((int64_t)s * sm.F + min(fs, sm.F - 1)) * C * B + nq;
#pragma unroll
    for (int c = 0; c < kBmSmC; ++c) sev[c] = *reinterpret_cast<const float4*>(ep + (int64_t)min(c, C - 1) * B);
#pragma unroll
    for (int j = 0; j < 4; ++j) yq[j] = sm.y[nq + j];
  }
  float4 rg[NA_], rp[NT_], rw[NT_], rt[NA_], rk[NT_];
  bm_load_mat<true>(Qb + 4, LD, M, tid, rg);
  bm_load_tile(Qb + NR, LD, M, n0, B, tid, rp);
  bm_load_tile(Wb, B, M, n0, B, tid, rw);
  const float av = tid < 128 ? Qb[(int64_t)min(tid, M - 1) * LD] : 0.f;
  const int ncl = min(n0 + (tid & 63), B - 1);
  float gmv = 0.f, gvv = 0.f;
  if (!sm.eps) { gmv = gmu[b * B + ncl]; gvv = gvar[b * B + ncl]; }
  bm_load_mat<true>(Tb, M, M, tid, rt);
  bm_load_tile(Kb, LD, M, n0, B, tid, rk);
  BM_STAMP(13);
  if (sm.eps) {
    const int cme = (int)(b % C);
    const float sc1 = 1.f / (float)(S * sm.F);
    float* smu = sP;
    float* ssd = sP + kBmSmC * 64;
    *reinterpret_cast<float4*>(&smu[fs * 64 + 4 * q4]) = mu4;
    *reinterpret_cast<float4*>(&ssd[fs * 64 + 4 * q4]) = make_float4(sqrtf(var4.x), sqrtf(var4.y), sqrtf(var4.z), sqrtf(var4.w));
    __syncthreads();
    float pm[4] = {0.f, 0.f, 0.f, 0.f}, pv[4] = {0.f, 0.f, 0.f, 0.f}, ct[4] = {0.f, 0.f, 0.f, 0.f};
    if (4 * wave < sm.F) {
      const bool live = n0 + 4 * q4 < B && fs < sm.F;
      const int yb[4] = {(int)yq[0], (int)yq[1], (int)yq[2], (int)yq[3]};
      float mx[4], fy[4] = {0.f, 0.f, 0.f, 0.f}, sdme[4] = {1.f, 1.f, 1.f, 1.f};
      float eme[4] = {0.f, 0.f, 0.f, 0.f};
#pragma unroll
      for (int j = 0; j < 4; ++j) mx[j] = -INFINITY;
#pragma unroll
      for (int cg = 0; cg < kBmSmC / 4; ++cg) {
        if (4 * cg >= C) continue;
#pragma unroll
        for (int c = 4 * cg; c < 4 * cg + 4; ++c) {
          const float4 m4 = *reinterpret_cast<const float4*>(&smu[c * 64 + 4 * q4]);
          const float4 s4 = *reinterpret_cast<const float4*>(&ssd[c * 64 + 4 * q4]);
          const float e[4] = {sev[c].x, sev[c].y, sev[c].z, sev[c].w};
          const float m_[4] = {m4.x, m4.y, m4.z, m4.w}, s_[4] = {s4.x, s4.y, s4.z, s4.w};
          float v[4];
#pragma unroll
          for (int j = 0; j < 4; ++j) {
            v[j] = c < C ? fmaf(s_[j], e[j], m_[j]) : -INFINITY;
            mx[j] = fmaxf(mx[j], v[j]);
            if (c == yb[j]) fy[j] = v[j];
            if (c == cme) { eme[j] = e[j]; sdme[j] = s_[j]; }
          }
          sev[c] = make_float4(v[0], v[1], v[2], v[3]);
        }
      }
      float se[4] = {0.f, 0.f, 0.f, 0.f}, vme[4] = {0.f, 0.f, 0.f, 0.f};
#pragma unroll
      for (int cg = 0; cg < kBmSmC / 4; ++cg) {
        if (4 * cg >= C) continue;
#pragma unroll
        for (int c = 4 * cg; c < 4 * cg + 4; ++c) {
          const float v[4] = {sev[c].x, sev[c].y, sev[c].z, sev[c].w};
#pragma unroll
          for (int j = 0; j < 4; ++j) {
            const float e = c < C ? expf(v[j] - mx[j]) : 0.f;
            se[j] += e;
            if (c == cme) vme[j] = e;
          }
        }
      }
#pragma unroll
      for (int j = 0; j < 4; ++j) {
        const float pc = vme[j] * (sc1 / se[j]) - (cme == yb[j] ? sc1 : 0.f);
        pm[j] = live ? pc : 0.f;
        pv[j] = live ? pc * eme[j] * (0.5f / sdme[j]) : 0.f;
        ct[j] = live ? -(fy[j] - (mx[j] + logf(se[j]))) * sc1 : 0.f;
      }
    }
#pragma unroll
    for (int j = 0; j < 4; ++j) {
      pm[j] += __shfl_xor(pm[j], 16, 64); pm[j] += __shfl_xor(pm[j], 32, 64);
      pv[j] += __shfl_xor(pv[j], 16, 64); pv[j] += __shfl_xor(pv[j], 32, 64);
      ct[j] += __shfl_xor(ct[j], 16, 64); ct[j] += __shfl_xor(ct[j], 32, 64);
    }
    BM_STAMP(14);
    float* sred = scs + 64 + 8;
    if (lane < 16) {
      *reinterpret_cast<float4*>(&sred[(0 * 4 + wave) * 64 + 4 * q4]) = make_float4(pm[0], pm[1], pm[2], pm[3]);
      *reinterpret_cast<float4*>(&sred[(1 * 4 + wave) * 64 + 4 * q4]) = make_float4(pv[0], pv[1], pv[2], pv[3]);
      *reinterpret_cast<float4*>(&sred[(2 * 4 + wave) * 64 + 4 * q4]) = make_float4(ct[0], ct[1], ct[2], ct[3]);
    }
    __syncthreads();
    BM_STAMP(15);
    if (tid < 64) {
      gmv = sred[tid] + sred[64 + tid] + sred[128 + tid] + sred[192 + tid];
      gvv = sred[256 + tid] + sred[320 + tid] + sred[384 + tid] + sred[448 + tid];
      if (cme == 0) {
        float t = sred[512 + tid] + sred[576 + tid] + sred[640 + tid] + sred[704 + tid];
        t = wave_sum(t);
        if (tid == 0) atomicAdd(sm.nll, t);
      }
    }
  }

  BM_STAMP(1);
  bm_store_mat<true>(sA, rg, M, tid);
  bm_store_tile(sP, rp, M, n0, B, tid);
  bm_store_tile(sW, rw, M, n0, B, tid);
  if (tid < 128) sa[tid] = tid < M ? av : 0.f;
  if (tid < 64) {
    const bool ok = n0 + tid < B;
    sgm[tid] = ok ? gs * gmv : 0.f;
    sgv[tid] = ok ? gs * gvv : 0.f;
    scs[tid] = 0.f;
  }
  __syncthreads();
  BM_STAMP(2);
  BM_CUT_AT(0);
#pragma unroll
  for (int u = 0; u < NT_; ++u) {
    const int e = tid + 256 * u;
    if (e < kBmKP * 16) {
      const int m = e >> 4, n = (e & 15) * 4;
      float4 w = *reinterpret_cast<const float4*>(&sW[m * kBmST + n]);
      const float4 g = *reinterpret_cast<const float4*>(&sgv[n]);
      w.x *= 2.f * g.x; w.y *= 2.f * g.y; w.z *= 2.f * g.z; w.w *= 2.f * g.w;
      *reinterpret_cast<float4*>(&sW[m * kBmST + n]) = w;
    }
  }
  {
    const int m = tid >> 1, h = tid & 1;
    const float* pr = sP + min(m, kBmKP - 1) * kBmST + 32 * h;
    float acc0 = 0.f, acc1 = 0.f;
#pragma unroll
    for (int i = 0; i < 8; ++i) {
      const float4 p = *reinterpret_cast<const float4*>(pr + 4 * i);
      const float4 g = *reinterpret_cast<const float4*>(&sgm[32 * h + 4 * i]);
      acc0 = fmaf(p.x, g.x, acc0); acc1 = fmaf(p.y, g.y, acc1); acc0 = fmaf(p.z, g.z, acc0); acc1 = fmaf(p.w, g.w, acc1);
    }
    float t = acc0 + acc1;
    t += __shfl_xor(t, 1, 64);
    if (h == 0 && m < M) atomicAdd(&gQP[b * MLD + (int64_t)m * LD], t);
    if (wave == 0) {
      const float tv = wave_sum(sgv[lane]);
      if (lane == 0) atomicAdd(&gkd[b], tv);
    }
  }
  __syncthreads();
  BM_STAMP(3);
  BM_CUT_AT(1);
  const int cbh = wave & 1;
  const int rbs[2] = {(wave >> 1) ? 1 : 0, (wave >> 1) ? 2 : 3};
  bm_f32x16 accP[2], accG[3];
  float* dG = gQP + b * MLD + 4;
  if (wave == 0) bm_phase2<0>(sA, sP, sW, sa, sgm, sgv, dG, LD, M, li, lh, accP, accG);
  else if (wave == 1) bm_phase2<1>(sA, sP, sW, sa, sgm, sgv, dG, LD, M, li, lh, accP, accG);
  else if (wave == 2) bm_phase2<2>(sA, sP, sW, sa, sgm, sgv, dG, LD, M, li, lh, accP, accG);
  else bm_phase2<3>(sA, sP, sW, sa, sgm, sgv, dG, LD, M, li, lh, accP, accG);
  BM_STAMP(4);
  BM_CUT_AT(2);
  BM_STAMP(5);
  bmm_lds_barrier();
  BM_STAMP(6);
  BM_CUT_AT(3);
#pragma unroll
  for (int u = 0; u < 2; ++u)
#pragma unroll
    for (int r = 0; r < 16; ++r) {
      const int m = 32 * rbs[u] + (r & 3) + 8 * (r >> 2) + 4 * lh;
      if (m < kBmKP) sP[m * kBmST + 32 * cbh + li] = m < M ? accP[u][r] : 0.f;
    }
  bm_store_mat<true>(sA, rt, M, tid);
  bm_store_tile(sW, rk, M, n0, B, tid);
  bmm_lds_barrier();
  BM_STAMP(7);
  BM_CUT_AT(4);
  {
    bm_f32x16 acc[2];
    bm_f32x16 accT[3];
    float* dT = gTT + b * MM;
    if (wave == 0) bm_phase4<0>(sA, sP, sW, dT, M, M, li, lh, acc, accG, dG, LD, accT);
    else if (wave == 1) bm_phase4<1>(sA, sP, sW, dT, M, M, li, lh, acc, accG, dG, LD, accT);
    else if (wave == 2) bm_phase4<2>(sA, sP, sW, dT, M, M, li, lh, acc, accG, dG, LD, accT);
    else bm_phase4<3>(sA, sP, sW, dT, M, M, li, lh, acc, accG, dG, LD, accT);
    BM_STAMP(8);
    BM_CUT_AT(5);
    const int rlo = rbs[0], rhi = rbs[1];
    const int n = 32 * cbh + li;
    BM_STAMP(9);
    if (wave == 0) bm_tail_atomics<0>(accT, dT, M, M, li, lh);
    else if (wave == 1) bm_tail_atomics<1>(accT, dT, M, M, li, lh);
    else if (wave == 2) bm_tail_atomics<2>(accT, dT, M, M, li, lh);
    else bm_tail_atomics<3>(accT, dT, M, M, li, lh);
    float wv[2][16];
#pragma unroll
    for (int u = 0; u < 2; ++u) {
      const int rb = u ? rhi : rlo;
#pragma unroll
      for (int r = 0; r < 16; ++r) {
        const int m = 32 * rb + (r & 3) + 8 * (r >> 2) + 4 * lh;
        wv[u][r] = m < M ? acc[u][r] * sW[min(m, kBmKP - 1) * kBmST + n] : 0.f;
      }
    }
    bmm_lds_barrier();
#pragma unroll
    for (int u = 0; u < 2; ++u) {
      const int rb = u ? rhi : rlo;
#pragma unroll
      for (int r = 0; r < 16; ++r) {
        const int m = 32 * rb + (r & 3) + 8 * (r >> 2) + 4 * lh;
        if (m < kBmKP) sP[m * kBmST + n] = wv[u][r];
      }
    }
  }
  BM_STAMP(10);
  bmm_lds_barrier();
  BM_STAMP(11);
  {
    float* Gout = gRK + b * MLD + NR + n0;
    float4 cs = make_float4(0.f, 0.f, 0.f, 0.f);
    const int n4 = (tid & 15) * 4;
    float4 wv4[kBmNT];
#pragma unroll
    for (int u = 0; u < kBmNT; ++u) {
      const int e = min(tid + 256 * u, kBmKP * 16 - 1);
      wv4[u] = *reinterpret_cast<const float4*>(&sP[(e >> 4) * kBmST + n4]);
    }
#pragma unroll
    for (int u = 0; u < kBmNT; ++u) {
      const int e = tid + 256 * u, m = e >> 4;
      if (e < kBmKP * 16) { cs.x += wv4[u].x; cs.y += wv4[u].y; cs.z += wv4[u].z; cs.w += wv4[u].w; }
      if (m < M && n0 + n4 < B) *reinterpret_cast<float4*>(&Gout[(int64_t)m * LD + n4]) = wv4[u];
    }
    atomicAdd(&scs[n4], cs.x); atomicAdd(&scs[n4 + 1], cs.y); atomicAdd(&scs[n4 + 2], cs.z); atomicAdd(&scs[n4 + 3], cs.w);
    const int m = tid >> 1, h = tid & 1;
    const float* pr = sP + min(m, kBmKP - 1) * kBmST + 32 * h;
    float a0 = 0.f, a1 = 0.f;
#pragma unroll
    for (int i = 0; i < 8; ++i) {
      const float4 v = *reinterpret_cast<const float4*>(pr + 4 * i);
      a0 += v.x + v.z; a1 += v.y + v.w;
    }
    float t = a0 + a1;
    t += __shfl_xor(t, 1, 64);
    if (h == 0 && m < M) atomicAdd(&r_uf[b * M + m], t);
  }
  bmm_lds_barrier();
  {
    const int s = (int)(b / C);
    float cv = 0.f;
    if (tid < 64) {
      cv = scs[tid];
      if (n0 + tid < B) atomicAdd(&c_uf[(int64_t)s * B + n0 + tid], cv);
    }
    if (wave == 0) {
      const float tot = wave_sum(cv);
      if (lane == 0) atomicAdd(&gtheta[(int64_t)s * (D + 1) + D], 2.f * tot);
    }
  }
  BM_STAMP(12);
}

}
```

vargp_amd/csrc/t0_bwd_mid_multi.h:

```cpp
#pragma once
#include "t0_bwd_mid.h"

namespace vargp {

#ifdef BM_STAMPS
__device__ unsigned long long g_bmm_stamps[4][24];
extern "C" void vargp_debug_bmm_stamps(unsigned long long* out) { (void)hipMemcpyFromSymbol(out, HIP_SYMBOL(g_bmm_stamps), sizeof(g_bmm_stamps)); }
#define BMM_STAMP(i) do { if ((threadIdx.x & 63) == 0 && blockIdx.x == (BM_STAMP_BLOCK) && (tile == tile0 + 1 || (i) >= 20)) g_bmm_stamps[threadIdx.x >> 6][i] = __builtin_amdgcn_s_memtime(); } while (0)
#else
#define BMM_STAMP(i) do { } while (0)
#endif

constexpr size_t kBwdMidMultiLdsBytes =
    sizeof(float) * (2 * kBmKP * kBmSA + 2 * kBmKP * kBmST + 128  + 64 + 64  + 64  + 8);

typedef float bm_f32x4 __attribute__((ext_vector_type(4)));
constexpr int kB16NB = 7;
__device__ __forceinline__ void b16_mfma4(bm_f32x4& acc, const float4 a, const float4 b) {
  acc = __builtin_amdgcn_mfma_f32_16x16x4f32(a.x, b.x, acc, 0, 0, 0);
  acc = __builtin_amdgcn_mfma_f32_16x16x4f32(a.y, b.y, acc, 0, 0, 0);
  acc = __builtin_amdgcn_mfma_f32_16x16x4f32(a.z, b.z, acc, 0, 0, 0);
  acc = __builtin_amdgcn_mfma_f32_16x16x4f32(a.w, b.w, acc, 0, 0, 0);
}
__device__ __forceinline__ float4 b16_mask(const float4 v, const bool ok) {
  return make_float4(ok ? v.x : 0.f, ok ? v.y : 0.f, ok ? v.z : 0.f, ok ? v.w : 0.f);
}
template <int WV> struct B16Tri {
  static constexpr int RA = 6 - WV, NA = 7 - WV, RB = WV > 0 ? WV - 1 : 0, NBk = WV;
  __host__ __device__ static constexpr int rb(int u) { return u < NA ? RA : RB; }
  __host__ __device__ static constexpr int cb(int u) { return u < NA ? u : u - NA; }
};
template <int WV>
__device__ __forceinline__ void b16_tri_acc(const float* __restrict__ sX, const float* __restrict__ sY, int l16, int q,
                                            bm_f32x4 (&acc)[kB16NB]) {
  using W = B16Tri<WV>;
  const float* xa = sX + min(16 * W::RA + l16, kBmKP - 1) * kBmST + 4 * q;
  const float* xb = sX + min(16 * W::RB + l16, kBmKP - 1) * kBmST + 4 * q;
  const float* yr[W::NA];
#pragma unroll
  for (int c = 0; c < W::NA; ++c) yr[c] = sY + min(16 * c + l16, kBmKP - 1) * kBmST + 4 * q;
  float4 nxa = bm_frag_kc(xa, 0), nxb = nxa, ny[W::NA];
  if constexpr (W::NBk > 0) nxb = bm_frag_kc(xb, 0);
#pragma unroll
  for (int c = 0; c < W::NA; ++c) ny[c] = bm_frag_kc(yr[c], 0);
  bm_for<0, 4>([&](auto gi) {
    constexpr int g = decltype(gi)::value;
    const float4 cxa = nxa, cxb = nxb;
    float4 cy[W::NA];
#pragma unroll
    for (int c = 0; c < W::NA; ++c) cy[c] = ny[c];
    if constexpr (g + 1 < 4) {
      nxa = bm_frag_kc(xa, 16 * (g + 1));
      if constexpr (W::NBk > 0) nxb = bm_frag_kc(xb, 16 * (g + 1));
#pragma unroll
      for (int c = 0; c < W::NA; ++c) ny[c] = bm_frag_kc(yr[c], 16 * (g + 1));
    }
#pragma unroll
    for (int c = 0; c < W::NA; ++c) b16_mfma4(acc[c], cxa, cy[c]);
#pragma unroll
    for (int c = 0; c < W::NBk; ++c) b16_mfma4(acc[W::NA + c], cxb, cy[c]);
  });
}
template <bool LOWER, int SA = kBmSA>
__device__ __forceinline__ void b16_prod(const float* __restrict__ sA, const float* __restrict__ sB, int cw, int l16, int q,
                                         bm_f32x4 (&acc)[kB16NB]) {
  const float* ap[kB16NB];
#pragma unroll
  for (int i = 0; i < kB16NB; ++i)
    ap[i] = LOWER ? sA + min(16 * i + l16, kBmKP - 1) * SA + 4 * q : sA + (4 * q) * SA + min(16 * i + l16, kBmKP - 1);
  const float* bcol = sB + (4 * q) * kBmST + 16 * cw + l16;
  auto afrag = [&](const int i, const int g) -> float4 {
    if (LOWER) return g == 6 ? b16_mask(bm_frag_kc(ap[i], 16 * g - (q >= 2 ? 8 : 0)), q < 2) : bm_frag_kc(ap[i], 16 * g);
    return g == 6 ? b16_mask(bm_frag_km(ap[i], 16 * g - (q >= 2 ? 8 : 0), SA), q < 2) : bm_frag_km(ap[i], 16 * g, SA);
  };
  auto bfrag = [&](const int g) -> float4 {
    return g == 6 ? b16_mask(bm_frag_km(bcol, 16 * g - (q >= 2 ? 8 : 0), kBmST), q < 2) : bm_frag_km(bcol, 16 * g, kBmST);
  };
  constexpr int G0 = 0, G1 = kB16NB;
  float4 nb = bfrag(G0), na[kB16NB];
#pragma unroll
  for (int i = 0; i < kB16NB; ++i) na[i] = (LOWER ? i >= G0 : i <= G0) ? afrag(i, G0) : make_float4(0.f, 0.f, 0.f, 0.f);
  bm_for<G0, G1>([&](auto gi) {
    constexpr int g = decltype(gi)::value;
    const float4 bb = nb;
    float4 ca[kB16NB];
#pragma unroll
    for (int i = 0; i < kB16NB; ++i) ca[i] = na[i];
    if constexpr (g + 1 < G1) {
      nb = bfrag(g + 1);
#pragma unroll
      for (int i = 0; i < kB16NB; ++i)
        if (LOWER ? i >= g + 1 : i <= g + 1) na[i] = afrag(i, g + 1);
    }
#pragma unroll
    for (int i = 0; i < kB16NB; ++i)
      if (LOWER ? i >= g : i <= g) b16_mfma4(acc[i], ca[i], bb);
  });
}
template <int WV, int A>
__device__ __forceinline__ void b16_tri_atomic(const bm_f32x4 (&acc)[kB16NB], float* __restrict__ dst, int ldd, int M, int l16, int q) {
  using W = B16Tri<WV>;
  constexpr int u = A / 4, r = A % 4, rb = W::rb(u), cb = W::cb(u);
  if (16 * rb + r < M) {
    const int row = 16 * rb + 4 * q + r, col = 16 * cb + l16;
    if (row < M && (rb != cb || col <= row)) atomicAdd(&dst[(int64_t)row * ldd + col], acc[u][r]);
  }
}
template <int WV>
__device__ __forceinline__ void b16_flush_tri(const bm_f32x4 (&acc)[kB16NB], float* __restrict__ dst, int ldd, int M, int l16, int q) {
  bm_for<0, 4 * kB16NB>([&](auto ai) { b16_tri_atomic<WV, decltype(ai)::value>(acc, dst, ldd, M, l16, q); });
}
__device__ __forceinline__ void b16_flush(const int wave, const bm_f32x4 (&acc)[kB16NB], float* __restrict__ dst, int ldd, int M,
                                          int l16, int q) {
  asm volatile("" : "+s"(M));
  if (wave == 0) b16_flush_tri<0>(acc, dst, ldd, M, l16, q);
  else if (wave == 1) b16_flush_tri<1>(acc, dst, ldd, M, l16, q);
  else if (wave == 2) b16_flush_tri<2>(acc, dst, ldd, M, l16, q);
  else b16_flush_tri<3>(acc, dst, ldd, M, l16, q);
}
__device__ __forceinline__ void b16_tri(const int wave, const float* __restrict__ sX, const float* __restrict__ sY, int l16, int q,
                                        bm_f32x4 (&acc)[kB16NB]) {
  if (wave == 0) b16_tri_acc<0>(sX, sY, l16, q, acc);
  else if (wave == 1) b16_tri_acc<1>(sX, sY, l16, q, acc);
  else if (wave == 2) b16_tri_acc<2>(sX, sY, l16, q, acc);
  else b16_tri_acc<3>(sX, sY, l16, q, acc);
}

__global__ __launch_bounds__(256) void t0_bwd_mid_multi_kernel(const float* __restrict__ TT, const float* __restrict__ QP,
                                                               const float* __restrict__ Wf, const float* __restrict__ RK,
                                                               const float* __restrict__ gmu, const float* __restrict__ gvar,
                                                               const float* __restrict__ gscale, float* __restrict__ gQP,
                                                               float* __restrict__ gTT, float* __restrict__ gRK,
                                                               float* __restrict__ gkd, float* __restrict__ r_uf,
                                                               float* __restrict__ c_uf, float* __restrict__ gtheta, int S, int C,
                                                               int M, int B, int D, int NR, int LD, int ntile, int nparts,
                                                               float* __restrict__ zero_out, int zero_n) {
  extern __shared__ __attribute__((aligned(16))) float bm_lds[];
  STEP_SPAN(t0, 4);
  if (blockIdx.x == 0 && zero_out)
    for (int i = threadIdx.x; i < zero_n; i += 256) zero_out[i] = 0.f;
  float* sG = bm_lds;
  float* sT = sG + kBmKP * kBmSA;
  float* sP = sT + kBmKP * kBmSA;
  float* sW = sP + kBmKP * kBmST;
  float* sa = sW + kBmKP * kBmST;
  float* sgm = sa + 128;
  float* sgv = sgm + 64;
  float* scs = sgv + 64;
  const int tid_k = threadIdx.x, tid = tid_k, lane = tid & 63, wave = tid >> 6;
  const int xcd = (int)blockIdx.x & 7, idx = (int)blockIdx.x >> 3;
  const int64_t b = (int64_t)(idx / nparts) * 8 + xcd;
  if (b >= (int64_t)S * C) return;
  const int part = idx % nparts;
  const int tile0 = (part * ntile) / nparts, tile1 = ((part + 1) * ntile) / nparts;
  const int64_t MM = (int64_t)M * M, MLD = (int64_t)M * LD;
  const float* Qb = QP + b * MLD;
  const float* Tb = TT + b * MM;
  const float* Wb = Wf + b * (int64_t)M * B;
  const float* Kb = RK + b * MLD + NR;
  const float gs = gscale ? gscale[0] : 1.f;
  const int s = (int)(b / C);
  constexpr int NA_ = kBmNA, NT_ = kBmNT;
  { [[maybe_unused]] const int tile = -9; BMM_STAMP(20); }

  float4 rp[NT_], rw[NT_], rk[NT_];
  float gmv, gvv;
  auto load_tiles = [&](const int n0, const int tid) {
    const int ncl = min(n0 + (tid & 63), B - 1);
    gmv = gmu[b * B + ncl]; gvv = gvar[b * B + ncl];
    bm_load_tile(Qb + NR, LD, M, n0, B, tid, rp);
    bm_load_tile(Wb, B, M, n0, B, tid, rw);
  };

  gmv = gvv = 0.f;
  load_tiles(tile0 * 64, tid);
  {
    float4 rg[NA_], rt[NA_];
    bm_load_mat<true>(Qb + 4, LD, M, tid, rg);
    bm_load_mat<true>(Tb, M, M, tid, rt);
    const float av = tid < 128 ? Qb[(int64_t)min(tid, M - 1) * LD] : 0.f;
    bm_store_mat<true>(sG, rg, M, tid);
    bm_store_mat<true>(sT, rt, M, tid);
    if (tid < 128) sa[tid] = tid < M ? av : 0.f;
  }
  { [[maybe_unused]] const int tile = -9; BMM_STAMP(21); }

  bm_f32x4 accG[kB16NB], accT[kB16NB];
#pragma unroll
  for (int u = 0; u < kB16NB; ++u)
#pragma unroll
    for (int r = 0; r < 4; ++r) { accG[u][r] = 0.f; accT[u][r] = 0.f; }
  float ga_acc = 0.f, ruf_acc = 0.f, gkd_acc = 0.f, gth_acc = 0.f;

  for (int tile = tile0; tile < tile1; ++tile) {
    const int n0 = tile * 64;
    int tid = tid_k;
    asm volatile("" : "+v"(tid));
    asm volatile("" : "+s"(M), "+s"(B), "+s"(LD), "+s"(NR), "+s"(C));
    const int lane = tid & 63, wave = tid >> 6, l16 = lane & 15, q = lane >> 4;
    const int n = 16 * wave + l16;
    BMM_STAMP(0);
    BMM_STAMP(1);
    bm_store_tile(sP, rp, M, n0, B, tid);
    bm_store_tile(sW, rw, M, n0, B, tid);
    BMM_STAMP(15);
    bm_load_tile(Kb, LD, M, n0, B, tid, rk);
    if (tid < 64) {
      const bool ok = n0 + tid < B;
      sgm[tid] = ok ? gs * gmv : 0.f;
      sgv[tid] = ok ? gs * gvv : 0.f;
      scs[tid] = 0.f;
    }
    bmm_lds_barrier();
    BMM_STAMP(2);
#pragma unroll
    for (int u = 0; u < NT_; ++u) {
      const int e = tid + 256 * u;
      if (e < kBmKP * 16) {
        const int m = e >> 4, n = (e & 15) * 4;
        float4 w = *reinterpret_cast<const float4*>(&sW[m * kBmST + n]);
        const float4 g = *reinterpret_cast<const float4*>(&sgv[n]);
        w.x *= 2.f * g.x; w.y *= 2.f * g.y; w.z *= 2.f * g.z; w.w *= 2.f * g.w;
        *reinterpret_cast<float4*>(&sW[m * kBmST + n]) = w;
      }
    }
    {
      const int m = tid >> 1, h = tid & 1;
      const float* pr = sP + min(m, kBmKP - 1) * kBmST + 32 * h;
      float acc0 = 0.f, acc1 = 0.f;
#pragma unroll
      for (int i = 0; i < 8; ++i) {
        const float4 p = *reinterpret_cast<const float4*>(pr + 4 * i);
        const float4 g = *reinterpret_cast<const float4*>(&sgm[32 * h + 4 * i]);
        acc0 = fmaf(p.x, g.x, acc0); acc1 = fmaf(p.y, g.y, acc1); acc0 = fmaf(p.z, g.z, acc0); acc1 = fmaf(p.w, g.w, acc1);
      }
      ga_acc += acc0 + acc1;
      if (wave == 0) gkd_acc += sgv[lane];
    }
    bmm_lds_barrier();
    BMM_STAMP(3);
    b16_tri(wave, sP, sW, l16, q, accG);
    bm_f32x4 accP[kB16NB];
    {
      const float gmn = sgm[n], gvn = sgv[n];
#pragma unroll
      for (int i = 0; i < kB16NB; ++i)
#pragma unroll
        for (int r = 0; r < 4; ++r) {
          const int m = 16 * i + 4 * q + r, mc = min(m, kBmKP - 1);
          accP[i][r] = m < kBmKP ? fmaf(sa[mc], gmn, -2.f * sP[mc * kBmST + n] * gvn) : 0.f;
        }
    }
    b16_prod<true>(sG, sW, wave, l16, q, accP);
    BMM_STAMP(4);
    if (tile + 1 == tile1) b16_flush(wave, accG, gQP + b * MLD + 4, LD, M, l16, q);
    bmm_lds_barrier();
    BMM_STAMP(5);
#pragma unroll
    for (int i = 0; i < kB16NB; ++i)
#pragma unroll
      for (int r = 0; r < 4; ++r) {
        const int m = 16 * i + 4 * q + r;
        if (m < kBmKP) sP[m * kBmST + n] = m < M ? accP[i][r] : 0.f;
      }
    bm_store_tile(sW, rk, M, n0, B, tid);
    if (tile + 1 < tile1) load_tiles(n0 + 64, tid);
    bmm_lds_barrier();
    BMM_STAMP(6);
    {
      b16_tri(wave, sP, sW, l16, q, accT);
      bm_f32x4 acc[kB16NB];
#pragma unroll
      for (int i = 0; i < kB16NB; ++i)
#pragma unroll
        for (int r = 0; r < 4; ++r) acc[i][r] = 0.f;
      b16_prod<false>(sT, sP, wave, l16, q, acc);
      BMM_STAMP(7);
      if (tile + 1 == tile1) b16_flush(wave, accT, gTT + b * MM, M, M, l16, q);
      float wv[kB16NB][4];
#pragma unroll
      for (int i = 0; i < kB16NB; ++i)
#pragma unroll
        for (int r = 0; r < 4; ++r) {
          const int m = 16 * i + 4 * q + r;
          wv[i][r] = m < M ? acc[i][r] * sW[min(m, kBmKP - 1) * kBmST + n] : 0.f;
        }
      BMM_STAMP(16);
      bmm_lds_barrier();
      BMM_STAMP(17);
#pragma unroll
      for (int i = 0; i < kB16NB; ++i)
#pragma unroll
        for (int r = 0; r < 4; ++r) {
          const int m = 16 * i + 4 * q + r;
          if (m < kBmKP) sP[m * kBmST + n] = wv[i][r];
        }
    }
    bmm_lds_barrier();
    BMM_STAMP(8);
    {
      float* Gout = gRK + b * MLD + NR + n0;
      float4 cs = make_float4(0.f, 0.f, 0.f, 0.f);
      const int n4 = (tid & 15) * 4;
      float4 wv4[kBmNT];
#pragma unroll
      for (int u = 0; u < kBmNT; ++u) {
        const int e = min(tid + 256 * u, kBmKP * 16 - 1);
        wv4[u] = *reinterpret_cast<const float4*>(&sP[(e >> 4) * kBmST + n4]);
      }
#pragma unroll
      for (int u = 0; u < kBmNT; ++u) {
        const int e = tid + 256 * u, m = e >> 4;
        if (e < kBmKP * 16) { cs.x += wv4[u].x; cs.y += wv4[u].y; cs.z += wv4[u].z; cs.w += wv4[u].w; }
        if (m < M && n0 + n4 < B) *reinterpret_cast<float4*>(&Gout[(int64_t)m * LD + n4]) = wv4[u];
      }
      atomicAdd(&scs[n4], cs.x); atomicAdd(&scs[n4 + 1], cs.y); atomicAdd(&scs[n4 + 2], cs.z); atomicAdd(&scs[n4 + 3], cs.w);
      const int m = tid >> 1, h = tid & 1;
      const float* pr = sP + min(m, kBmKP - 1) * kBmST + 32 * h;
      float a0 = 0.f, a1 = 0.f;
#pragma unroll
      for (int i = 0; i < 8; ++i) {
        const float4 v = *reinterpret_cast<const float4*>(pr + 4 * i);
        a0 += v.x + v.z; a1 += v.y + v.w;
      }
      ruf_acc += a0 + a1;
    }
    bmm_lds_barrier();
    BMM_STAMP(9);
    if (tid < 64) {
      const float cv = scs[tid];
      if (n0 + tid < B) atomicAdd(&c_uf[(int64_t)s * B + n0 + tid], cv);
      gth_acc += cv;
    }
    BMM_STAMP(10);
  }

  {
    const int m = tid >> 1, h = tid & 1;
    ga_acc += __shfl_xor(ga_acc, 1, 64);
    ruf_acc += __shfl_xor(ruf_acc, 1, 64);
    if (h == 0 && m < M) {
      atomicAdd(&gQP[b * MLD + (int64_t)m * LD], ga_acc);
      atomicAdd(&r_uf[b * M + m], ruf_acc);
    }
    if (wave == 0) {
      const float tv = wave_sum(gkd_acc);
      const float tot = wave_sum(gth_acc);
      if (lane == 0) {
        atomicAdd(&gkd[b], tv);
        atomicAdd(&gtheta[(int64_t)s * (D + 1) + D], 2.f * tot);
      }
    }
  }
  { [[maybe_unused]] const int tile = -9; BMM_STAMP(22); }
}

}
```

Baseline: 5381 ELBO steps/s (Cfg2 step: S=3 hyper-samples).

## Rework fused backward-mid kernel to 8 waves with 16x16 MFMA tiles

The single-tile fused backward-mid kernel moves from 256 threads (4 waves using 32x32x2 MFMA blocks) to 512 threads (8 waves using 16x16x4 MFMA blocks). Triangular and product work is redistributed across the wave sets with new row/column block tables, and the LDS reductions are adjusted to the new thread count. The aim is more latency hiding and finer load balance inside each block for the M=100 triangular products. The trade-off is more registers per block, a larger LDS scratch area, and possibly lower occupancy and extra barrier cost.

Measured after the change: 5415 ELBO steps/s (Cfg2 step: S=3 hyper-samples) (median of 6 runs). About the same (+0.6%).

```diff
diff --git a/vargp_amd/csrc/elbo_t0.hip b/vargp_amd/csrc/elbo_t0.hip
--- a/vargp_amd/csrc/elbo_t0.hip
+++ b/vargp_amd/csrc/elbo_t0.hip
@@ -728,6 +728,7 @@
   bool fused_bwd, mat_bwd, bwd_multi, fused_tail, tail_lds;
   int kuf_tile, puf_tile, puu_tile;
   int ksp, ntile, fwd_parts, bwd_parts;
+  int bwd_mid_threads;
 };
 static T0Plan t0_plan(const vargp_elbo_t0_desc* d, const T0Ws& o, int cus) {
   const T0Tune& tune = t0_tune();
@@ -763,6 +764,7 @@
   p.mat_bwd = p.fused_bwd && tune.mat_bwd && (D % 4) == 0 && S <= kTailSMax && zx_aligned;
   p.bwd_parts = t0_tile_parts(SC, p.ntile, cus, kBwdMidSetup, tune.parts);
   p.bwd_multi = p.fused_bwd && (p.bwd_parts < p.ntile || tune.multi == 1);
+  p.bwd_mid_threads = kBmThreads;
   p.defer_softmax = d->defer_softmax && p.unscaled_lik_grad && p.fused_bwd && !p.bwd_multi && F <= 4 * kBmSmF && C <= kBmSmC &&
                     reinterpret_cast<uintptr_t>(p.native ? o.eps_f : d->eps_f) % 16 == 0;
   p.fwd_softmax16 = p.unscaled_lik_grad && !p.defer_softmax;
@@ -1039,7 +1041,7 @@
       rc = ensure_dynamic_lds(reinterpret_cast<const void*>(t0_bwd_mid_kernel), kBwdMidLdsBytes, attr_set_mask, "elbo_t0_bwd");
       if (rc) return rc;
       ProfScope prof("t0_bwd_mid", st);
-      hipLaunchKernelGGL(t0_bwd_mid_kernel, dim3(8 * cdiv(SC, 8) * plan.ntile), dim3(256), kBwdMidLdsBytes, st, o.TT, o.QP, o.W, o.RK, o.gmu, o.gvar,
+      hipLaunchKernelGGL(t0_bwd_mid_kernel, dim3(8 * cdiv(SC, 8) * plan.ntile), dim3(plan.bwd_mid_threads), kBwdMidLdsBytes, st, o.TT, o.QP, o.W, o.RK, o.gmu, o.gvar,
                          lik_seed, o.gQP, o.gTT, o.gRK, o.gkd, o.r_uf, o.c_uf, o.gtheta, S, C, M, B, D,
                          NR, LD, plan.ntile, gum, C * M, smx);
     }
diff --git a/vargp_amd/csrc/t0_bwd_common.h b/vargp_amd/csrc/t0_bwd_common.h
--- a/vargp_amd/csrc/t0_bwd_common.h
+++ b/vargp_amd/csrc/t0_bwd_common.h
@@ -10,7 +10,8 @@
 constexpr int kBmST = 68;
 constexpr size_t kBwdMidLdsBytes =
     sizeof(float) * (kBmKP * kBmSA + 2 * kBmKP * kBmST + 128  + 64 + 64  + 64  + 8 +
-                     3 * 4 * 64 );
+                     3 * 8 * 64 );
+constexpr int kBmThreads = 512;
 constexpr int kBmSmC = 16, kBmSmF = 4;
 struct BmSoftmax {
   const float *mu, *var, *eps;
@@ -46,14 +47,15 @@
 __host__ __device__ constexpr int bm_min(int a, int b) { return a < b ? a : b; }
 
 constexpr int kBmNQ = kBmKP / 4;
-constexpr int kBmNA = (kBmKP * kBmNQ + 255) / 256;
+constexpr int bm_na(int nth) { return (kBmKP * kBmNQ + nth - 1) / nth; }
+constexpr int kBmNA = bm_na(256);
 
-template <bool TRI = false>
-__device__ __forceinline__ void bm_load_mat(const float* __restrict__ base, int ld, int M, int tid, float4 (&dst)[kBmNA]) {
+template <bool TRI = false, int NTH = 256>
+__device__ __forceinline__ void bm_load_mat(const float* __restrict__ base, int ld, int M, int tid, float4 (&dst)[bm_na(NTH)]) {
   const char* bp = reinterpret_cast<const char*>(base);
 #pragma unroll
-  for (int u = 0; u < kBmNA; ++u) {
-    const int e = min(tid + 256 * u, kBmKP * kBmNQ - 1);
+  for (int u = 0; u < bm_na(NTH); ++u) {
+    const int e = min(tid + NTH * u, kBmKP * kBmNQ - 1);
     const int i = e / kBmNQ, j = (e - i * kBmNQ) * 4;
     const int ic = min(i, M - 1);
     const int jc = TRI ? min(j, min(M - 4, ic & ~3)) : min(j, M - 4);
@@ -62,4 +64,16 @@
   }
 }
 
+typedef float bm_f32x4 __attribute__((ext_vector_type(4)));
+constexpr int kB16NB = 7;
+__device__ __forceinline__ void b16_mfma4(bm_f32x4& acc, const float4 a, const float4 b) {
+  acc = __builtin_amdgcn_mfma_f32_16x16x4f32(a.x, b.x, acc, 0, 0, 0);
+  acc = __builtin_amdgcn_mfma_f32_16x16x4f32(a.y, b.y, acc, 0, 0, 0);
+  acc = __builtin_amdgcn_mfma_f32_16x16x4f32(a.z, b.z, acc, 0, 0, 0);
+  acc = __builtin_amdgcn_mfma_f32_16x16x4f32(a.w, b.w, acc, 0, 0, 0);
 }
+__device__ __forceinline__ float4 b16_mask(const float4 v, const bool ok) {
+  return make_float4(ok ? v.x : 0.f, ok ? v.y : 0.f, ok ? v.z : 0.f, ok ? v.w : 0.f);
+}
+
+}
diff --git a/vargp_amd/csrc/t0_bwd_mid.h b/vargp_amd/csrc/t0_bwd_mid.h
--- a/vargp_amd/csrc/t0_bwd_mid.h
+++ b/vargp_amd/csrc/t0_bwd_mid.h
@@ -4,151 +4,194 @@
 namespace vargp {
 
 template <int WV> struct BmWave {
-  static constexpr int NB = WV < 2 ? 3 : 2;
-  static constexpr int R0 = WV < 2 ? 0 : 1, R1 = WV < 2 ? 3 : 2, CBH = WV & 1;
-  __host__ __device__ static constexpr int rb(int u) { return WV == 0 ? (u == 0 ? 0 : 1) : (WV == 1 ? 2 : 3); }
-  __host__ __device__ static constexpr int cb(int u) { return WV == 0 ? (u == 2 ? 1 : 0) : (WV == 1 ? u : (WV == 2 ? u : 2 + u)); }
+  static constexpr int NB = WV < 4 ? 4 : 3;
+  static constexpr int CW = WV & 3, SET = WV >> 2;
+  __host__ __device__ static constexpr int rb(int u) {
+    return WV == 0 ? 6 : WV == 1 ? 4 : WV == 2 ? 3 : WV == 3 ? (u < 2 ? 1 : (u == 2 ? 0 : 4)) : WV == 4 ? 6 : WV == 7 ? 2 : 5;
+  }
+  __host__ __device__ static constexpr int cb(int u) {
+    return WV == 3 ? (u == 1 ? 1 : (u == 3 ? 4 : 0)) : WV == 4 ? 4 + u : WV == 6 ? 3 + u : u;
+  }
 };
-
-__host__ __device__ constexpr int kBmAtomSplit(int nb) { return 8 * nb; }
-
-template <int WV>
-__device__ __forceinline__ void bm_tri_mfma(const float* __restrict__ sX, const float* __restrict__ sY, int li, int lh,
-                                            bm_f32x16 (&acc)[3]) {
+__host__ __device__ constexpr int bm_nrow(int set) { return set ? 3 : 4; }
+__host__ __device__ constexpr int bm_prow(bool lower, int set, int u) {
+  return lower ? (set ? (u == 0 ? 2 : (u == 1 ? 4 : 5)) : (u == 0 ? 0 : (u == 1 ? 1 : (u == 2 ? 3 : 6))))
+               : (set ? (u == 0 ? 1 : (u == 1 ? 2 : 4)) : (u == 0 ? 0 : (u == 1 ? 3 : (u == 2 ? 5 : 6))));
+}
+constexpr int kBmNBmax = 4;
+
+__host__ __device__ constexpr int kBmAtomSplit(int nb) { return 2 * nb; }
+
+__device__ __forceinline__ float bm_f4c(const float4 v, const int j) { return j == 0 ? v.x : (j == 1 ? v.y : (j == 2 ? v.z : v.w)); }
+
+template <int WV, class AF>
+__device__ __forceinline__ void bm_tri_mfma(const float* __restrict__ sX, const float* __restrict__ sY, int l16, int q,
+                                            bm_f32x4 (&acc)[kBmNBmax], AF&& after) {
   using W = BmWave<WV>;
-  const float* xr[3];
-  const float* yr[3];
-#pragma unroll
-  for (int u = 0; u < 3; ++u) {
-#pragma unroll
-    for (int r = 0; r < 16; ++r) acc[u][r] = 0.f;
-    xr[u] = sX + min(32 * W::rb(u < W::NB ? u : 0) + li, kBmKP - 1) * kBmST + 4 * lh;
-    yr[u] = sY + min(32 * W::cb(u < W::NB ? u : 0) + li, kBmKP - 1) * kBmST + 4 * lh;
-  }
-#pragma unroll
-  for (int k = 0; k < 64; k += 8) {
-#pragma unroll
-    for (int u = 0; u < W::NB; ++u) bm_mfma4(acc[u], bm_frag_kc(xr[u], k), bm_frag_kc(yr[u], k));
-  }
+  const float* xr[W::NB];
+  const float* yr[W::NB];
+  float4 nx[W::NB], ny[W::NB];
+#pragma unroll
+  for (int u = 0; u < kBmNBmax; ++u)
+#pragma unroll
+    for (int r = 0; r < 4; ++r) acc[u][r] = 0.f;
+#pragma unroll
+  for (int u = 0; u < W::NB; ++u) {
+    xr[u] = sX + min(16 * W::rb(u) + l16, kBmKP - 1) * kBmST + 4 * q;
+    yr[u] = sY + min(16 * W::cb(u) + l16, kBmKP - 1) * kBmST + 4 * q;
+    nx[u] = bm_frag_kc(xr[u], 0);
+    ny[u] = bm_frag_kc(yr[u], 0);
+  }
+  bm_for<0, 4>([&](auto gi) {
+    constexpr int g = decltype(gi)::value;
+    float4 cx[W::NB], cy[W::NB];
+#pragma unroll
+    for (int u = 0; u < W::NB; ++u) { cx[u] = nx[u]; cy[u] = ny[u]; }
+    if constexpr (g + 1 < 4) {
+#pragma unroll
+      for (int u = 0; u < W::NB; ++u) {
+        nx[u] = bm_frag_kc(xr[u], 16 * (g + 1));
+        ny[u] = bm_frag_kc(yr[u], 16 * (g + 1));
+      }
+    }
+#pragma unroll
+    for (int j = 0; j < 4; ++j)
+#pragma unroll
+      for (int u = 0; u < W::NB; ++u)
+        acc[u] = __builtin_amdgcn_mfma_f32_16x16x4f32(bm_f4c(cx[u], j), bm_f4c(cy[u], j), acc[u], 0, 0, 0);
+    after(gi);
+  });
 }
 template <int WV, int A>
-__device__ __forceinline__ void bm_tri_atomic(const bm_f32x16 (&acc)[3], float* __restrict__ dst, int ldd, int M, int li, int lh) {
+__device__ __forceinline__ void bm_tri_atomic(const bm_f32x4 (&acc)[kBmNBmax], float* __restrict__ dst, int ldd, int M, int l16, int q) {
   using W = BmWave<WV>;
-  constexpr int u = A / 16, r = A % 16, rb = W::rb(u), cb = W::cb(u);
-  constexpr int rl = (r & 3) + 8 * (r >> 2);
-  if (32 * rb + rl < M) {
-    const int row = 32 * rb + rl + 4 * lh, col = 32 * cb + li;
-    const bool ok = row < M && (rb != cb || col <= row);
-#ifndef BM_EXP_NOATOM
-#ifdef BM_EXP_PLAIN_STORES
-    if (ok) dst[(int64_t)row * ldd + col] = acc[u][r];
-#else
-    if (ok) atomicAdd(&dst[(int64_t)row * ldd + col], acc[u][r]);
-#endif
-#else
-    if (ok && acc[u][r] == 12345.f) dst[(int64_t)row * ldd + col] = 0.f;
-#endif
-  }
+  constexpr int u = A / 4, r = A % 4, rb = W::rb(u), cb = W::cb(u);
+  if (16 * rb + r < M) {
+    const int row = 16 * rb + 4 * q + r, col = 16 * cb + l16;
+    if (row < M && (rb != cb || col <= row)) atomicAdd(&dst[(int64_t)row * ldd + col], acc[u][r]);
+  }
+}
+
+template <bool LOWER, int SET> struct BmProd {
+  static constexpr int NR = bm_nrow(SET);
+  static constexpr int G0 = LOWER ? 0 : bm_prow(false, SET, 0), G1 = LOWER ? bm_prow(true, SET, NR - 1) + 1 : kB16NB, NG = G1 - G0;
+};
+template <bool LOWER, int SET, class AF>
+__device__ __forceinline__ void bm_prod(const float* __restrict__ sA, const float* __restrict__ sB, int cw, int l16, int q,
+                                        bm_f32x4 (&acc)[kBmNBmax], AF&& after) {
+  using PR = BmProd<LOWER, SET>;
+  constexpr int NR = PR::NR;
+  const float* ap[NR];
+#pragma unroll
+  for (int u = 0; u < NR; ++u) {
+    const int i = bm_prow(LOWER, SET, u);
+    ap[u] = LOWER ? sA + min(16 * i + l16, kBmKP - 1) * kBmSA + 4 * q : sA + (4 * q) * kBmSA + min(16 * i + l16, kBmKP - 1);
+  }
+  const float* bcol = sB + (4 * q) * kBmST + 16 * cw + l16;
+  auto afrag = [&](const int u, const int g) -> float4 {
+    if (LOWER) return g == 6 ? b16_mask(bm_frag_kc(ap[u], 16 * g - (q >= 2 ? 8 : 0)), q < 2) : bm_frag_kc(ap[u], 16 * g);
+    return g == 6 ? b16_mask(bm_frag_km(ap[u], 16 * g - (q >= 2 ? 8 : 0), kBmSA), q < 2) : bm_frag_km(ap[u], 16 * g, kBmSA);
+  };
+  auto bfrag = [&](const int g) -> float4 {
+    return g == 6 ? b16_mask(bm_frag_km(bcol, 16 * g - (q >= 2 ? 8 : 0), kBmST), q < 2) : bm_frag_km(bcol, 16 * g, kBmST);
+  };
+  auto active = [](const int u, const int g) { return LOWER ? bm_prow(LOWER, SET, u) >= g : bm_prow(LOWER, SET, u) <= g; };
+  float4 nb = bfrag(PR::G0), na[NR];
+#pragma unroll
+  for (int u = 0; u < NR; ++u) na[u] = active(u, PR::G0) ? afrag(u, PR::G0) : make_float4(0.f, 0.f, 0.f, 0.f);
+  bm_for<PR::G0, PR::G1>([&](auto gi) {
+    constexpr int g = decltype(gi)::value;
+    const float4 bb = nb;
+    float4 ca[NR];
+#pragma unroll
+    for (int u = 0; u < NR; ++u) ca[u] = na[u];
+    if constexpr (g + 1 < PR::G1) {
+      nb = bfrag(g + 1);
+#pragma unroll
+      for (int u = 0; u < NR; ++u)
+        if (active(u, g + 1)) na[u] = afrag(u, g + 1);
+    }
+#pragma unroll
+    for (int j = 0; j < 4; ++j)
+#pragma unroll
+      for (int u = 0; u < NR; ++u)
+        if (active(u, g)) acc[u] = __builtin_amdgcn_mfma_f32_16x16x4f32(bm_f4c(ca[u], j), bm_f4c(bb, j), acc[u], 0, 0, 0);
+    after(std::integral_constant<int, g - PR::G0>{});
+    __builtin_amdgcn_sched_barrier(0);
+  });
 }
 
 template <int WV>
 __device__ __forceinline__ void bm_phase2(const float* __restrict__ sA, const float* __restrict__ sP, const float* __restrict__ sW,
                                           const float* __restrict__ sa, const float* __restrict__ sgm,
-                                          const float* __restrict__ sgv, float* __restrict__ dst, int ldd, int M, int li, int lh,
-                                          bm_f32x16 (&accP)[2], bm_f32x16 (&acc)[3]) {
+                                          const float* __restrict__ sgv, float* __restrict__ dst, int ldd, int M, int l16, int q,
+                                          bm_f32x4 (&accP)[kBmNBmax], bm_f32x4 (&acc)[kBmNBmax]) {
   using W = BmWave<WV>;
-  bm_tri_mfma<WV>(sP, sW, li, lh, acc);
-  constexpr int R[2] = {W::R0, W::R1};
-  const int n = 32 * W::CBH + li;
+  using PR = BmProd<true, W::SET>;
+  bm_tri_mfma<WV>(sP, sW, l16, q, acc, [](auto) {});
+  const int n = 16 * W::CW + l16;
   {
     const float gmn = sgm[n], gvn = sgv[n];
 #pragma unroll
-    for (int u = 0; u < 2; ++u)
-#pragma unroll
-      for (int r = 0; r < 16; ++r) {
-        const int m = 32 * R[u] + (r & 3) + 8 * (r >> 2) + 4 * lh;
+    for (int u = 0; u < kBmNBmax; ++u)
+#pragma unroll
+      for (int r = 0; r < 4; ++r) {
+        const int m = 16 * bm_prow(true, W::SET, u < PR::NR ? u : 0) + 4 * q + r;
         const int mc = min(m, kBmKP - 1);
-        accP[u][r] = m < kBmKP ? fmaf(sa[mc], gmn, -2.f * sP[mc * kBmST + n] * gvn) : 0.f;
-      }
-  }
-  constexpr int G0 = bm_min(kBmKP, 32 * W::R0 + 32) / 8, G1 = bm_min(kBmKP, 32 * W::R1 + 32) / 8;
-  constexpr int NAT = kBmAtomSplit(W::NB), PER = (NAT + G1 - 1) / G1;
-  const float* arow0 = sA + min(32 * W::R0 + li, kBmKP - 1) * kBmSA + 4 * lh;
-  const float* arow1 = sA + min(32 * W::R1 + li, kBmKP - 1) * kBmSA + 4 * lh;
-  const float* bcol = sW + (4 * lh) * kBmST + n;
-  float4 nb = bm_frag_km(bcol, 0, kBmST), na0 = bm_frag_kc(arow0, 0), na1 = bm_frag_kc(arow1, 0);
-  bm_for<0, G1>([&](auto gi) {
-    constexpr int g = decltype(gi)::value;
-    const float4 bb = nb, a0 = na0, a1 = na1;
-    if constexpr (g + 1 < G1) {
-      nb = bm_frag_km(bcol, 8 * (g + 1), kBmST);
-      na1 = bm_frag_kc(arow1, 8 * (g + 1));
-      if constexpr (g + 1 < G0) na0 = bm_frag_kc(arow0, 8 * (g + 1));
-    }
-    bm_mfma4(accP[1], a1, bb);
-    if constexpr (g < G0) bm_mfma4(accP[0], a0, bb);
-    bm_for<g * PER, bm_min((g + 1) * PER, NAT)>([&](auto ai) { bm_tri_atomic<WV, decltype(ai)::value>(acc, dst, ldd, M, li, lh); });
-    __builtin_amdgcn_sched_barrier(0);
+        accP[u][r] = (u < PR::NR && m < kBmKP) ? fmaf(sa[mc], gmn, -2.f * sP[mc * kBmST + n] * gvn) : 0.f;
+      }
+  }
+  constexpr int NAT = kBmAtomSplit(W::NB), PER = (NAT + PR::NG - 1) / PR::NG;
+  bm_prod<true, W::SET>(sA, sW, W::CW, l16, q, accP, [&](auto iti) {
+    constexpr int it = decltype(iti)::value;
+    bm_for<it * PER, bm_min((it + 1) * PER, NAT)>([&](auto ai) { bm_tri_atomic<WV, decltype(ai)::value>(acc, dst, ldd, M, l16, q); });
   });
 }
 
 template <int WV>
 __device__ __forceinline__ void bm_phase4(const float* __restrict__ sA, const float* __restrict__ sP, const float* __restrict__ sW,
-                                          float* __restrict__ dst, int ldd, int M, int li, int lh, bm_f32x16 (&accK)[2],
-                                          const bm_f32x16 (&prev)[3], float* __restrict__ dprev, int ldprev, bm_f32x16 (&acc)[3]) {
+                                          float* __restrict__ dst, int ldd, int M, int l16, int q, bm_f32x4 (&accK)[kBmNBmax],
+                                          const bm_f32x4 (&prev)[kBmNBmax], float* __restrict__ dprev, int ldprev,
+                                          bm_f32x4 (&acc)[kBmNBmax]) {
   using W = BmWave<WV>;
+  using PR = BmProd<false, W::SET>;
   {
-    const float* xr[3];
-    const float* yr[3];
-#pragma unroll
-    for (int u = 0; u < 3; ++u) {
-#pragma unroll
-      for (int r = 0; r < 16; ++r) acc[u][r] = 0.f;
-      xr[u] = sP + min(32 * W::rb(u < W::NB ? u : 0) + li, kBmKP - 1) * kBmST + 4 * lh;
-      yr[u] = sW + min(32 * W::cb(u < W::NB ? u : 0) + li, kBmKP - 1) * kBmST + 4 * lh;
-    }
-    constexpr int A0 = kBmAtomSplit(W::NB), A1 = 16 * W::NB, PERP = (A1 - A0 + 7) / 8;
-    bm_for<0, 8>([&](auto gi) {
+    constexpr int A0 = kBmAtomSplit(W::NB), A1 = 4 * W::NB, PERP = (A1 - A0 + 3) / 4;
+    bm_tri_mfma<WV>(sP, sW, l16, q, acc, [&](auto gi) {
       constexpr int g = decltype(gi)::value;
-#pragma unroll
-      for (int u = 0; u < W::NB; ++u) bm_mfma4(acc[u], bm_frag_kc(xr[u], 8 * g), bm_frag_kc(yr[u], 8 * g));
       bm_for<A0 + g * PERP, bm_min(A0 + (g + 1) * PERP, A1)>(
-          [&](auto ai) { bm_tri_atomic<WV, decltype(ai)::value>(prev, dprev, ldprev, M, li, lh); });
+          [&](auto ai) { bm_tri_atomic<WV, decltype(ai)::value>(prev, dprev, ldprev, M, l16, q); });
     });
   }
 #pragma unroll
-  for (int u = 0; u < 2; ++u)
-#pragma unroll
-    for (int r = 0; r < 16; ++r) accK[u][r] = 0.f;
-  constexpr int GS0 = 4 * W::R0, GS1 = 4 * W::R1, GE = kBmKP / 8;
-  constexpr int NIT = GE - GS0, NAT = kBmAtomSplit(W::NB), PER = (NAT + NIT - 1) / NIT;
-  const int n = 32 * W::CBH + li;
-  const float* acol0 = sA + (4 * lh) * kBmSA + min(32 * W::R0 + li, kBmKP - 1);
-  const float* acol1 = sA + (4 * lh) * kBmSA + min(32 * W::R1 + li, kBmKP - 1);
-  const float* bcol = sP + (4 * lh) * kBmST + n;
-  float4 nb = bm_frag_km(bcol, 8 * GS0, kBmST), na0 = bm_frag_km(acol0, 8 * GS0, kBmSA), na1 = na0;
-  if constexpr (GS1 == GS0) na1 = bm_frag_km(acol1, 8 * GS0, kBmSA);
-  bm_for<GS0, GE>([&](auto gi) {
-    constexpr int g = decltype(gi)::value;
-    const float4 bb = nb, a0 = na0, a1 = na1;
-    if constexpr (g + 1 < GE) {
-      nb = bm_frag_km(bcol, 8 * (g + 1), kBmST);
-      na0 = bm_frag_km(acol0, 8 * (g + 1), kBmSA);
-      if constexpr (g + 1 >= GS1) na1 = bm_frag_km(acol1, 8 * (g + 1), kBmSA);
-    }
-    bm_mfma4(accK[0], a0, bb);
-    if constexpr (g >= GS1) bm_mfma4(accK[1], a1, bb);
-    constexpr int it = g - GS0;
-    bm_for<it * PER, bm_min((it + 1) * PER, NAT)>([&](auto ai) { bm_tri_atomic<WV, decltype(ai)::value>(acc, dst, ldd, M, li, lh); });
-    __builtin_amdgcn_sched_barrier(0);
+  for (int u = 0; u < kBmNBmax; ++u)
+#pragma unroll
+    for (int r = 0; r < 4; ++r) accK[u][r] = 0.f;
+  constexpr int NAT = kBmAtomSplit(W::NB), PER = (NAT + PR::NG - 1) / PR::NG;
+  bm_prod<false, W::SET>(sA, sP, W::CW, l16, q, accK, [&](auto iti) {
+    constexpr int it = decltype(iti)::value;
+    bm_for<it * PER, bm_min((it + 1) * PER, NAT)>([&](auto ai) { bm_tri_atomic<WV, decltype(ai)::value>(acc, dst, ldd, M, l16, q); });
   });
 }
 
 template <int WV>
-__device__ __forceinline__ void bm_tail_atomics(const bm_f32x16 (&acc)[3], float* __restrict__ dst, int ldd, int M, int li, int lh) {
+__device__ __forceinline__ void bm_tail_atomics(const bm_f32x4 (&acc)[kBmNBmax], float* __restrict__ dst, int ldd, int M, int l16, int q) {
   using W = BmWave<WV>;
-  bm_for<kBmAtomSplit(W::NB), 16 * W::NB>([&](auto ai) { bm_tri_atomic<WV, decltype(ai)::value>(acc, dst, ldd, M, li, lh); });
-}
+  bm_for<kBmAtomSplit(W::NB), 4 * W::NB>([&](auto ai) { bm_tri_atomic<WV, decltype(ai)::value>(acc, dst, ldd, M, l16, q); });
+}
+#define BM_WAVE_SWITCH(wave, CALL)                                                                                          \
+  do {                                                                                                                        \
+    switch (wave) {                                                                                                           \
+      case 0: CALL(0); break;                                                                                                 \
+      case 1: CALL(1); break;                                                                                                 \
+      case 2: CALL(2); break;                                                                                                 \
+      case 3: CALL(3); break;                                                                                                 \
+      case 4: CALL(4); break;                                                                                                 \
+      case 5: CALL(5); break;                                                                                                 \
+      case 6: CALL(6); break;                                                                                                 \
+      default: CALL(7); break;                                                                                                \
+    }                                                                                                                         \
+  } while (0)
 
 #ifdef BM_STAMPS
 __device__ unsigned long long g_bm_stamps[16];
@@ -166,53 +209,57 @@
 #define BM_CUT_AT(i) do { } while (0)
 #endif
 
-constexpr int kBmNT = (kBmKP * 16 + 255) / 256;
-
+constexpr int bm_nt(int nth) { return (kBmKP * 16 + nth - 1) / nth; }
+constexpr int kBmNT = bm_nt(256);
+
+template <int NTH = 256>
 __device__ __forceinline__ void bm_load_tile(const float* __restrict__ base, int ld, int M, int n0, int B, int tid,
-                                             float4 (&dst)[kBmNT]) {
+                                             float4 (&dst)[bm_nt(NTH)]) {
   const char* bp = reinterpret_cast<const char*>(base);
 #pragma unroll
-  for (int u = 0; u < kBmNT; ++u) {
-    const int e = min(tid + 256 * u, kBmKP * 16 - 1);
+  for (int u = 0; u < bm_nt(NTH); ++u) {
+    const int e = min(tid + NTH * u, kBmKP * 16 - 1);
     const int m = e >> 4, n = (e & 15) * 4;
     const unsigned off = 4u * (__umul24((unsigned)min(m, M - 1), (unsigned)ld) + (unsigned)min(n0 + n, B - 4));
     dst[u] = *reinterpret_cast<const float4*>(bp + off);
   }
 }
-__device__ __forceinline__ void bm_store_tile(float* __restrict__ dst, const float4 (&src)[kBmNT], int M, int n0, int B, int tid) {
-#pragma unroll
-  for (int u = 0; u < kBmNT; ++u) {
-    const int e = tid + 256 * u;
+template <int NTH = 256>
+__device__ __forceinline__ void bm_store_tile(float* __restrict__ dst, const float4 (&src)[bm_nt(NTH)], int M, int n0, int B, int tid) {
+#pragma unroll
+  for (int u = 0; u < bm_nt(NTH); ++u) {
+    const int e = tid + NTH * u;
     const int m = e >> 4, n = (e & 15) * 4;
     const float4 v = (m < M && n0 + n < B) ? src[u] : make_float4(0.f, 0.f, 0.f, 0.f);
     if (e < kBmKP * 16) *reinterpret_cast<float4*>(&dst[m * kBmST + n]) = v;
   }
 }
 
-template <bool TRI = false>
-__device__ __forceinline__ void bm_store_mat(float* __restrict__ dst, const float4 (&src)[kBmNA], int M, int tid) {
-#pragma unroll
-  for (int u = 0; u < kBmNA; ++u) {
-    const int e = tid + 256 * u;
+template <bool TRI = false, int NTH = 256>
+__device__ __forceinline__ void bm_store_mat(float* __restrict__ dst, const float4 (&src)[bm_na(NTH)], int M, int tid) {
+#pragma unroll
+  for (int u = 0; u < bm_na(NTH); ++u) {
+    const int e = tid + NTH * u;
     const int i = e / kBmNQ, j = (e - i * kBmNQ) * 4;
     const float4 v = (i < M && j < M && (!TRI || j <= i)) ? src[u] : make_float4(0.f, 0.f, 0.f, 0.f);
     if (e < kBmKP * kBmNQ) *reinterpret_cast<float4*>(&dst[i * kBmSA + j]) = v;
   }
 }
 
-__global__ __launch_bounds__(256) void t0_bwd_mid_kernel(const float* __restrict__ TT, const float* __restrict__ QP,
-                                                         const float* __restrict__ Wf, const float* __restrict__ RK,
-                                                         const float* __restrict__ gmu, const float* __restrict__ gvar,
-                                                         const float* __restrict__ gscale, float* __restrict__ gQP,
-                                                         float* __restrict__ gTT, float* __restrict__ gRK,
-                                                         float* __restrict__ gkd, float* __restrict__ r_uf,
-                                                         float* __restrict__ c_uf, float* __restrict__ gtheta, int S, int C,
-                                                         int M, int B, int D, int NR, int LD, int ntile,
-                                                         float* __restrict__ zero_out, int zero_n, const BmSoftmax sm) {
+__global__ __launch_bounds__(kBmThreads) void t0_bwd_mid_kernel(const float* __restrict__ TT, const float* __restrict__ QP,
+                                                                const float* __restrict__ Wf, const float* __restrict__ RK,
+                                                                const float* __restrict__ gmu, const float* __restrict__ gvar,
+                                                                const float* __restrict__ gscale, float* __restrict__ gQP,
+                                                                float* __restrict__ gTT, float* __restrict__ gRK,
+                                                                float* __restrict__ gkd, float* __restrict__ r_uf,
+                                                                float* __restrict__ c_uf, float* __restrict__ gtheta, int S, int C,
+                                                                int M, int B, int D, int NR, int LD, int ntile,
+                                                                float* __restrict__ zero_out, int zero_n, const BmSoftmax sm) {
   extern __shared__ __attribute__((aligned(16))) float bm_lds[];
   STEP_SPAN(t0, 4);
+  constexpr int NTH = kBmThreads;
   if (blockIdx.x == 0 && zero_out)
-    for (int i = threadIdx.x; i < zero_n; i += 256) zero_out[i] = 0.f;
+    for (int i = threadIdx.x; i < zero_n; i += NTH) zero_out[i] = 0.f;
   float* sA = bm_lds;
   float* sP = sA + kBmKP * kBmSA;
   float* sW = sP + kBmKP * kBmST;
@@ -220,7 +267,7 @@
   float* sgm = sa + 128;
   float* sgv = sgm + 64;
   float* scs = sgv + 64;
-  const int tid = threadIdx.x, lane = tid & 63, wave = tid >> 6, li = lane & 31, lh = lane >> 5;
+  const int tid = threadIdx.x, lane = tid & 63, wave = __builtin_amdgcn_readfirstlane(tid >> 6), l16 = lane & 15, q = lane >> 4;
   const int xcd = (int)blockIdx.x & 7, idx = (int)blockIdx.x >> 3;
   const int64_t b = (int64_t)(idx / ntile) * 8 + xcd;
   if (b >= (int64_t)S * C) return;
@@ -231,79 +278,75 @@
   const float* Wb = Wf + b * (int64_t)M * B;
   const float* Kb = RK + b * MLD + NR;
   const float gs = gscale ? gscale[0] : 1.f;
-  constexpr int NA_ = kBmNA, NT_ = kBmNT;
+  constexpr int NA_ = bm_na(NTH), NT_ = bm_nt(NTH);
   BM_STAMP(0);
-  const int q4 = tid & 15, fs = tid >> 4;
-  const int nq = min(n0 + 4 * q4, B - 4);
-  float4 sev[kBmSmC], mu4 = make_float4(0.f, 0.f, 0.f, 0.f), var4 = mu4;
-  int64_t yq[4] = {0, 0, 0, 0};
+  const int cp = tid & 31, fs = tid >> 5;
+  const int nq = min(n0 + 2 * cp, B - 2);
+  float2 sev[kBmSmC], mu2 = make_float2(0.f, 0.f), var2 = mu2;
+  int64_t yq[2] = {0, 0};
   if (sm.eps) {
     const int s = (int)(b / C);
     const int64_t rc = ((int64_t)s * C + min(fs, C - 1)) * B + nq;
-    mu4 = *reinterpret_cast<const float4*>(sm.mu + rc);
-    var4 = *reinterpret_cast<const float4*>(sm.var + rc);
+    mu2 = *reinterpret_cast<const float2*>(sm.mu + rc);
+    var2 = *reinterpret_cast<const float2*>(sm.var + rc);
     const float* ep = sm.eps + ((int64_t)s * sm.F + min(fs, sm.F - 1)) * C * B + nq;
 #pragma unroll
-    for (int c = 0; c < kBmSmC; ++c) sev[c] = *reinterpret_cast<const float4*>(ep + (int64_t)min(c, C - 1) * B);
-#pragma unroll
-    for (int j = 0; j < 4; ++j) yq[j] = sm.y[nq + j];
+    for (int c = 0; c < kBmSmC; ++c) sev[c] = *reinterpret_cast<const float2*>(ep + (int64_t)min(c, C - 1) * B);
+#pragma unroll
+    for (int j = 0; j < 2; ++j) yq[j] = sm.y[nq + j];
   }
   float4 rg[NA_], rp[NT_], rw[NT_], rt[NA_], rk[NT_];
-  bm_load_mat<true>(Qb + 4, LD, M, tid, rg);
-  bm_load_tile(Qb + NR, LD, M, n0, B, tid, rp);
-  bm_load_tile(Wb, B, M, n0, B, tid, rw);
+  bm_load_mat<true, NTH>(Qb + 4, LD, M, tid, rg);
+  bm_load_tile<NTH>(Qb + NR, LD, M, n0, B, tid, rp);
+  bm_load_tile<NTH>(Wb, B, M, n0, B, tid, rw);
   const float av = tid < 128 ? Qb[(int64_t)min(tid, M - 1) * LD] : 0.f;
   const int ncl = min(n0 + (tid & 63), B - 1);
   float gmv = 0.f, gvv = 0.f;
   if (!sm.eps) { gmv = gmu[b * B + ncl]; gvv = gvar[b * B + ncl]; }
-  bm_load_mat<true>(Tb, M, M, tid, rt);
-  bm_load_tile(Kb, LD, M, n0, B, tid, rk);
+  bm_load_mat<true, NTH>(Tb, M, M, tid, rt);
+  bm_load_tile<NTH>(Kb, LD, M, n0, B, tid, rk);
   BM_STAMP(13);
   if (sm.eps) {
     const int cme = (int)(b % C);
     const float sc1 = 1.f / (float)(S * sm.F);
     float* smu = sP;
     float* ssd = sP + kBmSmC * 64;
-    *reinterpret_cast<float4*>(&smu[fs * 64 + 4 * q4]) = mu4;
-    *reinterpret_cast<float4*>(&ssd[fs * 64 + 4 * q4]) = make_float4(sqrtf(var4.x), sqrtf(var4.y), sqrtf(var4.z), sqrtf(var4.w));
-    __syncthreads();
-    float pm[4] = {0.f, 0.f, 0.f, 0.f}, pv[4] = {0.f, 0.f, 0.f, 0.f}, ct[4] = {0.f, 0.f, 0.f, 0.f};
-    if (4 * wave < sm.F) {
-      const bool live = n0 + 4 * q4 < B && fs < sm.F;
-      const int yb[4] = {(int)yq[0], (int)yq[1], (int)yq[2], (int)yq[3]};
-      float mx[4], fy[4] = {0.f, 0.f, 0.f, 0.f}, sdme[4] = {1.f, 1.f, 1.f, 1.f};
-      float eme[4] = {0.f, 0.f, 0.f, 0.f};
-#pragma unroll
-      for (int j = 0; j < 4; ++j) mx[j] = -INFINITY;
+    *reinterpret_cast<float2*>(&smu[fs * 64 + 2 * cp]) = mu2;
+    *reinterpret_cast<float2*>(&ssd[fs * 64 + 2 * cp]) = make_float2(sqrtf(var2.x), sqrtf(var2.y));
+    bmm_lds_barrier();
+    float pm[2] = {0.f, 0.f}, pv[2] = {0.f, 0.f}, ct[2] = {0.f, 0.f};
+    if (2 * wave < sm.F) {
+      const bool live = n0 + 2 * cp < B && fs < sm.F;
+      const int yb[2] = {(int)yq[0], (int)yq[1]};
+      float mx[2] = {-INFINITY, -INFINITY}, fy[2] = {0.f, 0.f}, sdme[2] = {1.f, 1.f}, eme[2] = {0.f, 0.f};
 #pragma unroll
       for (int cg = 0; cg < kBmSmC / 4; ++cg) {
         if (4 * cg >= C) continue;
 #pragma unroll
         for (int c = 4 * cg; c < 4 * cg + 4; ++c) {
-          const float4 m4 = *reinterpret_cast<const float4*>(&smu[c * 64 + 4 * q4]);
-          const float4 s4 = *reinterpret_cast<const float4*>(&ssd[c * 64 + 4 * q4]);
-          const float e[4] = {sev[c].x, sev[c].y, sev[c].z, sev[c].w};
-          const float m_[4] = {m4.x, m4.y, m4.z, m4.w}, s_[4] = {s4.x, s4.y, s4.z, s4.w};
-          float v[4];
-#pragma unroll
-          for (int j = 0; j < 4; ++j) {
+          const float2 m2 = *reinterpret_cast<const float2*>(&smu[c * 64 + 2 * cp]);
+          const float2 s2 = *reinterpret_cast<const float2*>(&ssd[c * 64 + 2 * cp]);
+          const float e[2] = {sev[c].x, sev[c].y}, m_[2] = {m2.x, m2.y}, s_[2] = {s2.x, s2.y};
+          float v[2];
+#pragma unroll
+          for (int j = 0; j < 2; ++j) {
             v[j] = c < C ? fmaf(s_[j], e[j], m_[j]) : -INFINITY;
             mx[j] = fmaxf(mx[j], v[j]);
             if (c == yb[j]) fy[j] = v[j];
             if (c == cme) { eme[j] = e[j]; sdme[j] = s_[j]; }
           }
-          sev[c] = make_float4(v[0], v[1], v[2], v[3]);
+          sev[c] = make_float2(v[0], v[1]);
         }
       }
-      float se[4] = {0.f, 0.f, 0.f, 0.f}, vme[4] = {0.f, 0.f, 0.f, 0.f};
+      float se[2] = {0.f, 0.f}, vme[2] = {0.f, 0.f};
 #pragma unroll
       for (int cg = 0; cg < kBmSmC / 4; ++cg) {
         if (4 * cg >= C) continue;
 #pragma unroll
         for (int c = 4 * cg; c < 4 * cg + 4; ++c) {
-          const float v[4] = {sev[c].x, sev[c].y, sev[c].z, sev[c].w};
-#pragma unroll
-          for (int j = 0; j < 4; ++j) {
+          const float v[2] = {sev[c].x, sev[c].y};
+#pragma unroll
+          for (int j = 0; j < 2; ++j) {
             const float e = c < C ? expf(v[j] - mx[j]) : 0.f;
             se[j] += e;
             if (c == cme) vme[j] = e;
@@ -311,7 +354,7 @@
         }
       }
 #pragma unroll
-      for (int j = 0; j < 4; ++j) {
+      for (int j = 0; j < 2; ++j) {
         const float pc = vme[j] * (sc1 / se[j]) - (cme == yb[j] ? sc1 : 0.f);
         pm[j] = live ? pc : 0.f;
         pv[j] = live ? pc * eme[j] * (0.5f / sdme[j]) : 0.f;
@@ -319,25 +362,30 @@
       }
     }
 #pragma unroll
-    for (int j = 0; j < 4; ++j) {
-      pm[j] += __shfl_xor(pm[j], 16, 64); pm[j] += __shfl_xor(pm[j], 32, 64);
-      pv[j] += __shfl_xor(pv[j], 16, 64); pv[j] += __shfl_xor(pv[j], 32, 64);
-      ct[j] += __shfl_xor(ct[j], 16, 64); ct[j] += __shfl_xor(ct[j], 32, 64);
+    for (int j = 0; j < 2; ++j) {
+      pm[j] += __shfl_xor(pm[j], 32, 64);
+      pv[j] += __shfl_xor(pv[j], 32, 64);
+      ct[j] += __shfl_xor(ct[j], 32, 64);
     }
     BM_STAMP(14);
     float* sred = scs + 64 + 8;
-    if (lane < 16) {
-      *reinterpret_cast<float4*>(&sred[(0 * 4 + wave) * 64 + 4 * q4]) = make_float4(pm[0], pm[1], pm[2], pm[3]);
-      *reinterpret_cast<float4*>(&sred[(1 * 4 + wave) * 64 + 4 * q4]) = make_float4(pv[0], pv[1], pv[2], pv[3]);
-      *reinterpret_cast<float4*>(&sred[(2 * 4 + wave) * 64 + 4 * q4]) = make_float4(ct[0], ct[1], ct[2], ct[3]);
-    }
-    __syncthreads();
+    if (lane < 32) {
+      *reinterpret_cast<float2*>(&sred[(0 * 8 + wave) * 64 + 2 * cp]) = make_float2(pm[0], pm[1]);
+      *reinterpret_cast<float2*>(&sred[(1 * 8 + wave) * 64 + 2 * cp]) = make_float2(pv[0], pv[1]);
+      *reinterpret_cast<float2*>(&sred[(2 * 8 + wave) * 64 + 2 * cp]) = make_float2(ct[0], ct[1]);
+    }
+    bmm_lds_barrier();
     BM_STAMP(15);
     if (tid < 64) {
-      gmv = sred[tid] + sred[64 + tid] + sred[128 + tid] + sred[192 + tid];
-      gvv = sred[256 + tid] + sred[320 + tid] + sred[384 + tid] + sred[448 + tid];
+      float t = 0.f;
+      gmv = gvv = 0.f;
+#pragma unroll
+      for (int w = 0; w < 8; ++w) {
+        gmv += sred[(0 * 8 + w) * 64 + tid];
+        gvv += sred[(1 * 8 + w) * 64 + tid];
+        t += sred[(2 * 8 + w) * 64 + tid];
+      }
       if (cme == 0) {
-        float t = sred[512 + tid] + sred[576 + tid] + sred[640 + tid] + sred[704 + tid];
         t = wave_sum(t);
         if (tid == 0) atomicAdd(sm.nll, t);
       }
@@ -345,9 +393,9 @@
   }
 
   BM_STAMP(1);
-  bm_store_mat<true>(sA, rg, M, tid);
-  bm_store_tile(sP, rp, M, n0, B, tid);
-  bm_store_tile(sW, rw, M, n0, B, tid);
+  bm_store_mat<true, NTH>(sA, rg, M, tid);
+  bm_store_tile<NTH>(sP, rp, M, n0, B, tid);
+  bm_store_tile<NTH>(sW, rw, M, n0, B, tid);
   if (tid < 128) sa[tid] = tid < M ? av : 0.f;
   if (tid < 64) {
     const bool ok = n0 + tid < B;
@@ -355,12 +403,12 @@
     sgv[tid] = ok ? gs * gvv : 0.f;
     scs[tid] = 0.f;
   }
-  __syncthreads();
+  bmm_lds_barrier();
   BM_STAMP(2);
   BM_CUT_AT(0);
 #pragma unroll
   for (int u = 0; u < NT_; ++u) {
-    const int e = tid + 256 * u;
+    const int e = tid + NTH * u;
     if (e < kBmKP * 16) {
       const int m = e >> 4, n = (e & 15) * 4;
       float4 w = *reinterpret_cast<const float4*>(&sW[m * kBmST + n]);
@@ -370,34 +418,34 @@
     }
   }
   {
-    const int m = tid >> 1, h = tid & 1;
-    const float* pr = sP + min(m, kBmKP - 1) * kBmST + 32 * h;
+    const int m = tid >> 2, h = tid & 3;
+    const float* pr = sP + min(m, kBmKP - 1) * kBmST + 16 * h;
     float acc0 = 0.f, acc1 = 0.f;
 #pragma unroll
-    for (int i = 0; i < 8; ++i) {
+    for (int i = 0; i < 4; ++i) {
       const float4 p = *reinterpret_cast<const float4*>(pr + 4 * i);
-      const float4 g = *reinterpret_cast<const float4*>(&sgm[32 * h + 4 * i]);
+      const float4 g = *reinterpret_cast<const float4*>(&sgm[16 * h + 4 * i]);
       acc0 = fmaf(p.x, g.x, acc0); acc1 = fmaf(p.y, g.y, acc1); acc0 = fmaf(p.z, g.z, acc0); acc1 = fmaf(p.w, g.w, acc1);
     }
     float t = acc0 + acc1;
     t += __shfl_xor(t, 1, 64);
+    t += __shfl_xor(t, 2, 64);
     if (h == 0 && m < M) atomicAdd(&gQP[b * MLD + (int64_t)m * LD], t);
     if (wave == 0) {
       const float tv = wave_sum(sgv[lane]);
       if (lane == 0) atomicAdd(&gkd[b], tv);
     }
   }
-  __syncthreads();
+  bmm_lds_barrier();
   BM_STAMP(3);
   BM_CUT_AT(1);
-  const int cbh = wave & 1;
-  const int rbs[2] = {(wave >> 1) ? 1 : 0, (wave >> 1) ? 2 : 3};
-  bm_f32x16 accP[2], accG[3];
+  const int n = 16 * (wave & 3) + l16;
+  const int set = wave >> 2;
+  bm_f32x4 accP[kBmNBmax], accG[kBmNBmax];
   float* dG = gQP + b * MLD + 4;
-  if (wave == 0) bm_phase2<0>(sA, sP, sW, sa, sgm, sgv, dG, LD, M, li, lh, accP, accG);
-  else if (wave == 1) bm_phase2<1>(sA, sP, sW, sa, sgm, sgv, dG, LD, M, li, lh, accP, accG);
-  else if (wave == 2) bm_phase2<2>(sA, sP, sW, sa, sgm, sgv, dG, LD, M, li, lh, accP, accG);
-  else bm_phase2<3>(sA, sP, sW, sa, sgm, sgv, dG, LD, M, li, lh, accP, accG);
+#define BM_CALL(WV) bm_phase2<WV>(sA, sP, sW, sa, sgm, sgv, dG, LD, M, l16, q, accP, accG)
+  BM_WAVE_SWITCH(wave, BM_CALL);
+#undef BM_CALL
   BM_STAMP(4);
   BM_CUT_AT(2);
   BM_STAMP(5);
@@ -405,54 +453,48 @@
   BM_STAMP(6);
   BM_CUT_AT(3);
 #pragma unroll
-  for (int u = 0; u < 2; ++u)
-#pragma unroll
-    for (int r = 0; r < 16; ++r) {
-      const int m = 32 * rbs[u] + (r & 3) + 8 * (r >> 2) + 4 * lh;
-      if (m < kBmKP) sP[m * kBmST + 32 * cbh + li] = m < M ? accP[u][r] : 0.f;
-    }
-  bm_store_mat<true>(sA, rt, M, tid);
-  bm_store_tile(sW, rk, M, n0, B, tid);
+  for (int u = 0; u < kBmNBmax; ++u)
+#pragma unroll
+    for (int r = 0; r < 4; ++r) {
+      const int m = 16 * (set ? bm_prow(true, 1, u < 3 ? u : 0) : bm_prow(true, 0, u)) + 4 * q + r;
+      if (u < bm_nrow(set) && m < kBmKP) sP[m * kBmST + n] = m < M ? accP[u][r] : 0.f;
+    }
+  bm_store_mat<true, NTH>(sA, rt, M, tid);
+  bm_store_tile<NTH>(sW, rk, M, n0, B, tid);
   bmm_lds_barrier();
   BM_STAMP(7);
   BM_CUT_AT(4);
   {
-    bm_f32x16 acc[2];
-    bm_f32x16 accT[3];
+    bm_f32x4 acc[kBmNBmax], accT[kBmNBmax];
     float* dT = gTT + b * MM;
-    if (wave == 0) bm_phase4<0>(sA, sP, sW, dT, M, M, li, lh, acc, accG, dG, LD, accT);
-    else if (wave == 1) bm_phase4<1>(sA, sP, sW, dT, M, M, li, lh, acc, accG, dG, LD, accT);
-    else if (wave == 2) bm_phase4<2>(sA, sP, sW, dT, M, M, li, lh, acc, accG, dG, LD, accT);
-    else bm_phase4<3>(sA, sP, sW, dT, M, M, li, lh, acc, accG, dG, LD, accT);
+#define BM_CALL(WV) bm_phase4<WV>(sA, sP, sW, dT, M, M, l16, q, acc, accG, dG, LD, accT)
+    BM_WAVE_SWITCH(wave, BM_CALL);
+#undef BM_CALL
     BM_STAMP(8);
     BM_CUT_AT(5);
-    const int rlo = rbs[0], rhi = rbs[1];
-    const int n = 32 * cbh + li;
     BM_STAMP(9);
-    if (wave == 0) bm_tail_atomics<0>(accT, dT, M, M, li, lh);
-    else if (wave == 1) bm_tail_atomics<1>(accT, dT, M, M, li, lh);
-    else if (wave == 2) bm_tail_atomics<2>(accT, dT, M, M, li, lh);
-    else bm_tail_atomics<3>(accT, dT, M, M, li, lh);
-    float wv[2][16];
-#pragma unroll
-    for (int u = 0; u < 2; ++u) {
-      const int rb = u ? rhi : rlo;
-#pragma unroll
-      for (int r = 0; r < 16; ++r) {
-        const int m = 32 * rb + (r & 3) + 8 * (r >> 2) + 4 * lh;
+#define BM_CALL(WV) bm_tail_atomics<WV>(accT, dT, M, M, l16, q)
+    BM_WAVE_SWITCH(wave, BM_CALL);
+#undef BM_CALL
+    float wv[kBmNBmax][4];
+    int mrow[kBmNBmax];
+#pragma unroll
+    for (int u = 0; u < kBmNBmax; ++u) {
+      mrow[u] = 16 * (set ? bm_prow(false, 1, u < 3 ? u : 0) : bm_prow(false, 0, u)) + 4 * q;
+#pragma unroll
+      for (int r = 0; r < 4; ++r) {
+        const int m = mrow[u] + r;
         wv[u][r] = m < M ? acc[u][r] * sW[min(m, kBmKP - 1) * kBmST + n] : 0.f;
       }
     }
     bmm_lds_barrier();
 #pragma unroll
-    for (int u = 0; u < 2; ++u) {
-      const int rb = u ? rhi : rlo;
-#pragma unroll
-      for (int r = 0; r < 16; ++r) {
-        const int m = 32 * rb + (r & 3) + 8 * (r >> 2) + 4 * lh;
-        if (m < kBmKP) sP[m * kBmST + n] = wv[u][r];
-      }
-    }
+    for (int u = 0; u < kBmNBmax; ++u)
+#pragma unroll
+      for (int r = 0; r < 4; ++r) {
+        const int m = mrow[u] + r;
+        if (u < bm_nrow(set) && m < kBmKP) sP[m * kBmST + n] = wv[u][r];
+      }
   }
   BM_STAMP(10);
   bmm_lds_barrier();
@@ -461,29 +503,30 @@
     float* Gout = gRK + b * MLD + NR + n0;
     float4 cs = make_float4(0.f, 0.f, 0.f, 0.f);
     const int n4 = (tid & 15) * 4;
-    float4 wv4[kBmNT];
-#pragma unroll
-    for (int u = 0; u < kBmNT; ++u) {
-      const int e = min(tid + 256 * u, kBmKP * 16 - 1);
+    float4 wv4[NT_];
+#pragma unroll
+    for (int u = 0; u < NT_; ++u) {
+      const int e = min(tid + NTH * u, kBmKP * 16 - 1);
       wv4[u] = *reinterpret_cast<const float4*>(&sP[(e >> 4) * kBmST + n4]);
     }
 #pragma unroll
-    for (int u = 0; u < kBmNT; ++u) {
-      const int e = tid + 256 * u, m = e >> 4;
+    for (int u = 0; u < NT_; ++u) {
+      const int e = tid + NTH * u, m = e >> 4;
       if (e < kBmKP * 16) { cs.x += wv4[u].x; cs.y += wv4[u].y; cs.z += wv4[u].z; cs.w += wv4[u].w; }
       if (m < M && n0 + n4 < B) *reinterpret_cast<float4*>(&Gout[(int64_t)m * LD + n4]) = wv4[u];
     }
     atomicAdd(&scs[n4], cs.x); atomicAdd(&scs[n4 + 1], cs.y); atomicAdd(&scs[n4 + 2], cs.z); atomicAdd(&scs[n4 + 3], cs.w);
-    const int m = tid >> 1, h = tid & 1;
-    const float* pr = sP + min(m, kBmKP - 1) * kBmST + 32 * h;
+    const int m = tid >> 2, h = tid & 3;
+    const float* pr = sP + min(m, kBmKP - 1) * kBmST + 16 * h;
     float a0 = 0.f, a1 = 0.f;
 #pragma unroll
-    for (int i = 0; i < 8; ++i) {
+    for (int i = 0; i < 4; ++i) {
       const float4 v = *reinterpret_cast<const float4*>(pr + 4 * i);
       a0 += v.x + v.z; a1 += v.y + v.w;
     }
     float t = a0 + a1;
     t += __shfl_xor(t, 1, 64);
+    t += __shfl_xor(t, 2, 64);
     if (h == 0 && m < M) atomicAdd(&r_uf[b * M + m], t);
   }
   bmm_lds_barrier();
diff --git a/vargp_amd/csrc/t0_bwd_mid_multi.h b/vargp_amd/csrc/t0_bwd_mid_multi.h
--- a/vargp_amd/csrc/t0_bwd_mid_multi.h
+++ b/vargp_amd/csrc/t0_bwd_mid_multi.h
@@ -14,17 +14,6 @@
 constexpr size_t kBwdMidMultiLdsBytes =
     sizeof(float) * (2 * kBmKP * kBmSA + 2 * kBmKP * kBmST + 128  + 64 + 64  + 64  + 8);
 
-typedef float bm_f32x4 __attribute__((ext_vector_type(4)));
-constexpr int kB16NB = 7;
-__device__ __forceinline__ void b16_mfma4(bm_f32x4& acc, const float4 a, const float4 b) {
-  acc = __builtin_amdgcn_mfma_f32_16x16x4f32(a.x, b.x, acc, 0, 0, 0);
-  acc = __builtin_amdgcn_mfma_f32_16x16x4f32(a.y, b.y, acc, 0, 0, 0);
-  acc = __builtin_amdgcn_mfma_f32_16x16x4f32(a.z, b.z, acc, 0, 0, 0);
-  acc = __builtin_amdgcn_mfma_f32_16x16x4f32(a.w, b.w, acc, 0, 0, 0);
-}
-__device__ __forceinline__ float4 b16_mask(const float4 v, const bool ok) {
-  return make_float4(ok ? v.x : 0.f, ok ? v.y : 0.f, ok ? v.z : 0.f, ok ? v.w : 0.f);
-}
 template <int WV> struct B16Tri {
   static constexpr int RA = 6 - WV, NA = 7 - WV, RB = WV > 0 ? WV - 1 : 0, NBk = WV;
   __host__ __device__ static constexpr int rb(int u) { return u < NA ? RA : RB; }
```
